# empymod/emg3d

Measured on AMD Instinct MI355X. Metric: Mcells/s per multigrid cycle, higher is better.
Workload: dtype c128

## Files before the change

### emg3d_amd/_lib.py

```python
import ctypes
import os

import numpy as np

_HERE = os.path.dirname(os.path.abspath(__file__))
LIB_PATH = os.environ.get("EMG3D_HIP_LIB") or os.path.join(_HERE, "libemg3d_hip.so")
LAB_PATH = os.path.join(_HERE, "libemg3d_hip_lab.so")

c_i64 = ctypes.c_int64
c_int = ctypes.c_int
c_vp = ctypes.c_void_p
c_double = ctypes.c_double
c_dp = ctypes.POINTER(ctypes.c_double)

ABI_VERSION = 109

SIGNATURES = {
    "emg3d_hip_version": (c_int, []),
    "emg3d_hip_device_count": (c_int, [ctypes.POINTER(c_int)]),
    "emg3d_hip_set_device": (c_int, [c_int]),
    "emg3d_hip_device_info": (c_int, [c_int, ctypes.c_char_p, ctypes.POINTER(c_i64), ctypes.POINTER(c_int)]),
    "emg3d_hip_mem_info": (c_int, [c_int, ctypes.POINTER(c_i64), ctypes.POINTER(c_i64)]),
    "emg3d_hip_release_cached": (c_i64, []),
    "emg3d_hip_cached_bytes": (c_i64, []),
    "emg3d_hip_cached_bytes_on": (c_i64, [c_int]),
    "emg3d_mg_placement": (c_int, [c_vp, c_int, ctypes.POINTER(c_int), ctypes.POINTER(c_int), ctypes.POINTER(ctypes.c_float)]),
    "emg3d_amat_x": (c_int, [c_int, c_i64, c_i64, c_i64, c_vp, c_vp, c_vp, c_vp, c_vp, c_vp, c_vp, c_vp, c_vp]),
    "emg3d_get_h_field": (c_int, [c_int, c_i64, c_i64, c_i64, c_vp, c_vp, c_vp, c_vp, c_vp, c_vp, c_double, c_double]),
    "emg3d_gauss_seidel": (c_int, [c_int, c_int, c_i64, c_i64, c_i64, c_vp, c_vp, c_vp, c_vp, c_vp, c_vp,
                                   c_vp, c_vp, c_vp, c_int, c_int]),
    "emg3d_restrict": (c_int, [c_int, c_i64, c_i64, c_i64, c_i64, c_i64, c_i64, c_vp, c_vp, c_vp, c_int]),
    "emg3d_restrict_weights": (c_int, [c_vp, c_vp, c_vp, c_i64, c_vp, c_vp, c_vp, c_i64, c_vp, c_vp, c_vp]),
    "emg3d_solve": (c_int, [c_int, c_vp, c_vp, c_i64]),
    "emg3d_blocks_to_amat": (c_int, [c_int, c_vp, c_vp, c_i64, c_vp, c_vp, c_vp, c_i64, c_i64]),
    "emg3d_prolongation": (c_int, [c_int, c_i64, c_i64, c_i64, c_vp, c_vp, c_vp, c_vp, c_vp, c_vp, c_int]),
    "emg3d_restrict_model": (c_int, [c_int, c_i64, c_i64, c_i64, c_vp, c_vp, c_int]),
    "emg3d_sweep_plan": (c_int, [c_int, c_i64, c_i64, c_i64, c_int, c_int, c_int, c_int, ctypes.c_char_p, ctypes.POINTER(c_i64)]),
    "emg3d_mg_create": (c_int, [ctypes.POINTER(c_vp), c_int, c_i64, c_i64, c_i64, c_vp, c_vp, c_vp, c_vp,
                                c_vp, c_vp, c_vp, c_vp, c_int]),
    "emg3d_mg_destroy": (None, [c_vp]),
    "emg3d_mg_create_sv": (c_int, [ctypes.POINTER(c_vp), c_int, c_i64, c_i64, c_i64, c_vp, c_vp, c_vp, c_vp,
                                   c_vp, c_vp, c_vp, c_vp, c_double, c_double, c_int]),
    "emg3d_mg_create_vs": (c_int, [ctypes.POINTER(c_vp), c_int, c_i64, c_i64, c_i64, c_vp, c_vp, c_vp, c_vp,
                                   c_vp, c_vp, c_vp, c_vp, c_vp, c_double, c_double, c_int, c_int]),
    "emg3d_mg_create_vse": (c_int, [ctypes.POINTER(c_vp), c_int, c_i64, c_i64, c_i64, c_vp, c_vp, c_vp, c_vp,
                                    c_vp, c_vp, c_vp, c_vp, c_vp, c_vp, c_double, c_double, c_double, c_int, c_int]),
    "emg3d_mg_set_smu0_eps": (c_int, [c_vp, c_double, c_double, c_double]),
    "emg3d_mg_set_sfield_vector": (c_int, [c_vp, c_vp, c_double, c_double]),
    "emg3d_mg_set_sfield_dipole": (c_int, [c_vp, c_vp, c_vp, c_int, c_int, c_vp]),
    "emg3d_source_field": (c_int, [c_int, c_i64, c_i64, c_i64, c_vp, c_vp, c_vp, c_vp, c_vp, c_vp, c_int, c_vp, c_vp]),
    "emg3d_mg_prepare": (c_int, [c_vp, c_int, c_int]),
    "emg3d_mg_set_trace": (c_int, [c_vp, c_int]),
    "emg3d_mg_get_trace": (c_int, [c_vp, c_int, c_vp, c_vp, c_vp]),
    "emg3d_mg_set_params": (c_int, [c_vp, c_int, c_int, c_int, c_int, c_int, c_vp, c_int]),
    "emg3d_mg_set_sfield": (c_int, [c_vp, c_vp]),
    "emg3d_mg_set_efield": (c_int, [c_vp, c_vp]),
    "emg3d_mg_get_efield": (c_int, [c_vp, c_vp]),
    "emg3d_mg_get_residual": (c_int, [c_vp, c_vp]),
    "emg3d_mg_get_hfield": (c_int, [c_vp, c_int, c_double, c_double, c_vp]),
    "emg3d_interp3d": (c_int, [c_int, c_i64, c_i64, c_i64, c_vp, c_vp, c_vp, c_vp, c_i64, c_vp, c_int, c_int, c_double,
                               c_double, c_vp]),
    "emg3d_get_receiver_response": (c_int, [c_int, c_i64, c_i64, c_i64, c_vp, c_vp, c_vp, c_vp, c_vp, c_int, c_i64,
                                            c_vp, c_vp, c_vp]),
    "emg3d_mg_get_receiver_response": (c_int, [c_vp, c_int, c_int, c_double, c_double, c_i64, c_vp, c_vp, c_vp]),
    "emg3d_edges2cellaverages": (c_int, [c_int, c_i64, c_i64, c_i64, c_vp, c_vp, c_vp, c_vp, c_vp]),
    "emg3d_mg_gradient": (c_int, [c_vp, c_int, c_double, c_double, c_vp]),
    "emg3d_mg_gradient3": (c_int, [c_vp, c_int, c_double, c_double, c_vp, c_vp, c_vp]),
    "emg3d_mg_grad_acc_reset": (c_int, [c_vp]),
    "emg3d_mg_grad_acc_add": (c_int, [c_vp, c_int, c_double, c_double, c_vp]),
    "emg3d_mg_grad_acc_get": (c_int, [c_vp, c_vp]),
    "emg3d_mg_grad_acc3_reset": (c_int, [c_vp]),
    "emg3d_mg_grad_acc3_add": (c_int, [c_vp, c_int, c_double, c_double, c_vp]),
    "emg3d_mg_grad_acc3_get": (c_int, [c_vp, c_vp, c_vp, c_vp]),
    "emg3d_cells2edges": (c_int, [c_int, c_i64, c_i64, c_i64, c_vp, c_vp, c_vp, c_vp, c_vp, c_vp, c_vp]),
    "emg3d_mg_jvec_source": (c_int, [c_vp, c_int, c_double, c_double, c_vp, c_vp, c_vp]),
    "emg3d_mg_jvec_source_b": (c_int, [c_vp, c_int, c_double, c_double, c_vp, c_vp, c_vp, c_vp]),
    "emg3d_mg_get_receiver_response_linear": (c_int, [c_vp, c_i64, c_vp, c_vp, c_vp]),
    "emg3d_mg_set_receiver_adjoint": (c_int, [c_vp, c_i64, c_vp, c_vp, c_vp, c_int]),
    "emg3d_mg_get_receiver_response_linear_h": (c_int, [c_vp, c_double, c_double, c_i64, c_vp, c_vp, c_vp]),
    "emg3d_mg_set_receiver_adjoint_ex": (c_int, [c_vp, c_int, c_int, c_double, c_double, c_i64, c_vp, c_vp, c_vp, c_int]),
    "emg3d_mg_set_receiver_adjoint_b": (c_int, [c_vp, c_int, c_int, c_double, c_double, c_i64, c_vp, c_vp, c_vp, c_vp, c_int]),
    "emg3d_receiver_adjoint": (c_int, [c_int, c_i64, c_i64, c_i64, c_vp, c_vp, c_vp, c_vp, c_int, c_int, c_double, c_double,
                                       c_i64, c_vp, c_vp, c_vp, c_vp]),
    "emg3d_volume_average_weights": (c_int, [c_vp, c_i64, c_vp, c_i64, c_vp, c_vp, c_vp, c_vp, c_vp]),
    "emg3d_volume_average": (c_int, [c_int, c_i64, c_i64, c_i64, c_vp, c_vp, c_vp, c_vp, c_i64, c_i64, c_i64, c_vp, c_vp,
                                     c_vp, c_vp, c_vp]),
    "emg3d_interp3d_grid": (c_int, [c_int, c_i64, c_i64, c_i64, c_vp, c_vp, c_vp, c_vp, c_i64, c_vp, c_i64, c_vp, c_i64,
                                    c_vp, c_int, c_int, c_double, c_double, c_vp]),
    "emg3d_mg_set_batch": (c_int, [c_vp, c_int]),
    "emg3d_mg_get_batch": (c_int, [c_vp]),
    "emg3d_mg_select": (c_int, [c_vp, c_int]),
    "emg3d_mg_set_mask": (c_int, [c_vp, c_vp]),
    "emg3d_mg_residual_norm": (c_int, [c_vp, c_dp]),
    "emg3d_mg_sfield_norm": (c_int, [c_vp, c_dp]),
    "emg3d_mg_smooth": (c_int, [c_vp, c_int, c_int]),
    "emg3d_mg_begin": (c_int, [c_vp, c_int]),
    "emg3d_mg_set_smu0": (c_int, [c_vp, ctypes.c_double, ctypes.c_double]),
    "emg3d_mg_cycle": (c_int, [c_vp, c_int, c_int, c_dp]),
    "emg3d_mg_cycle_next": (c_int, [c_vp, c_int, c_int, c_int, c_int, c_dp]),
    "emg3d_mg_cycles": (c_int, [c_vp, c_int, c_vp, c_int, c_vp, c_int, c_vp]),
    "emg3d_mg_efield_devptr": (c_vp, [c_vp]),
    "emg3d_mg_sfield_devptr": (c_vp, [c_vp]),
    "emg3d_mg_stream": (c_vp, [c_vp]),
    "emg3d_mg_nE": (c_i64, [c_vp]),
    "emg3d_mg_sync": (c_int, [c_vp]),
    "emg3d_mg_device_bytes": (c_i64, [c_vp]),
    "emg3d_mg_time_sweep": (c_int, [c_vp, c_int, c_int, ctypes.POINTER(ctypes.c_float)]),
    "emg3d_mg_last_sweep_kernel": (c_int, [c_vp, ctypes.c_char_p]),
    "emg3d_mg_time_residual": (c_int, [c_vp, c_int, ctypes.POINTER(ctypes.c_float)]),
    "emg3d_mg_last_residual_kernel": (c_int, [c_vp, ctypes.c_char_p]),
    "emg3d_mg_amatvec": (c_int, [c_vp, c_vp, c_vp]),
    "emg3d_mg_vec_alloc": (c_int, [c_vp, c_int]),
    "emg3d_mg_vec_set": (c_int, [c_vp, c_int, c_vp]),
    "emg3d_mg_vec_get": (c_int, [c_vp, c_int, c_vp]),
    "emg3d_mg_vec_copy": (c_int, [c_vp, c_int, c_int]),
    "emg3d_mg_vec_axpy": (c_int, [c_vp, c_int, c_double, c_double, c_int]),
    "emg3d_mg_vec_scale": (c_int, [c_vp, c_int, c_double, c_double]),
    "emg3d_mg_vec_dot": (c_int, [c_vp, c_int, c_int, c_dp]),
    "emg3d_mg_vec_amatvec": (c_int, [c_vp, c_int, c_int]),
    "emg3d_mg_bvec_alloc": (c_int, [c_vp, c_int]),
# ... 25 lines not shown
            "  python -c 'import __graft_entry__ as g; g.build()'   (needs hipcc)\n"
            "emg3d_amd has no CPU fallback.")
    lib = ctypes.CDLL(path)
    try:
        lib.emg3d_hip_version.restype = c_int
        got = int(lib.emg3d_hip_version())
    except AttributeError:
        got = None
    if got != ABI_VERSION:
        raise HipLibraryError(
            f"{path} has ABI version {got}, this package needs {ABI_VERSION} (include/emg3d_hip.h: EMG3D_HIP_ABI_VERSION): "
            "a stale build. Rebuild it with\n  python -c 'import __graft_entry__ as g; g.build(force=True)'")
    for name, (res, args) in SIGNATURES.items():
        fn = getattr(lib, name)
        fn.restype = res
        fn.argtypes = args
    _loaded[path] = lib
    return lib


def load():
    global _lib, _path
    if _lib is None:
        _lib, _path = _open(LIB_PATH), LIB_PATH
    return _lib


def use(path=None):
    global _lib, _path
    prev = _path or LIB_PATH
    want = path or LIB_PATH
    _lib, _path = _open(want), want
    return prev


def check(status, what):
    if status != 0:
        raise HipLibraryError(f"{what} failed with status {status} "
                              f"({'invalid argument' if status < 0 else 'HIP error'})")


def dtype_code(dtype):
    dtype = np.dtype(dtype)
    if dtype == np.complex128:
        return 1
    if dtype == np.float64:
        return 0
    raise TypeError(f"fields must be float64 or complex128, got {dtype}")


def ptr(a):
    return a.ctypes.data_as(c_vp)


def device_count():
    n = c_int(0)
    check(load().emg3d_hip_device_count(ctypes.byref(n)), "emg3d_hip_device_count")
    return n.value


def device_info(device=0):
    name = ctypes.create_string_buffer(256)
    mem = c_i64(0)
    cus = c_int(0)
    check(load().emg3d_hip_device_info(device, name, ctypes.byref(mem), ctypes.byref(cus)),
          "emg3d_hip_device_info")
    return {"name": name.value.decode(), "total_mem": mem.value, "cu_count": cus.value}


def mem_info(device=0):
    fr, tot = c_i64(0), c_i64(0)
    check(load().emg3d_hip_mem_info(device, ctypes.byref(fr), ctypes.byref(tot)), "emg3d_hip_mem_info")
    return {"free": fr.value, "total": tot.value, "pooled": int(load().emg3d_hip_cached_bytes()),
            "pooled_on_device": int(load().emg3d_hip_cached_bytes_on(device))}


def sweep_plan(vnC, direction, dtype=np.complex128, ordering='colour', nsys=1, cu_count=0):
    name = ctypes.create_string_buffer(64)
    info = (c_i64 * 6)()
    check(load().emg3d_sweep_plan(dtype_code(dtype), int(vnC[0]), int(vnC[1]), int(vnC[2]), int(direction),
                                  1 if ordering == 'colour' else 0, int(nsys), int(cu_count), name, info), "emg3d_sweep_plan")
    return {"kernel": name.value.decode(), "lines_per_colour": info[0], "lines_per_wave": info[1], "rounds": info[2],
            "factor_kind": info[3], "split": bool(info[4]), "big_offsets": bool(info[5])}
```

### emg3d_amd/csrc/emg3d_hip.hip

```cpp
#include "../../include/emg3d_hip.h"

#include <cstring>
#include <new>

#include <chrono>
#include "mg.hpp"
#include "receivers.hpp"
#include "source.hpp"
#include "gradient.hpp"
#include "regrid.hpp"

#define EMG3D_HIP_VERSION EMG3D_HIP_ABI_VERSION

namespace {

template <class T>
MG<T>* as(emg3d_mg_t* mg) { return static_cast<MG<T>*>(reinterpret_cast<emg3d_mg*>(mg)); }

static int current_device() { int d = 0; if (hipGetDevice(&d) != hipSuccess) { (void)hipGetLastError(); d = 0; } return d; }

template <class T> static T scalar_of(double re, double im);
template <> double scalar_of<double>(double re, double) { return re; }
template <> c128 scalar_of<c128>(double re, double im) { return mk(re, im); }

// ... 408 lines not shown
template <class T>
void receiver_components(const std::vector<double> nodes[3], const std::vector<double> centers[3], const i64 nC[3],
                         bool electric, const T* field_dev, RcvComp<T> comp[3]) {
    i64 o = 0;
    for (int c = 0; c < 3; ++c) {
        comp[c].dev = field_dev + o;
        i64 tot = 1;
        for (int a = 0; a < 3; ++a) {
            const bool cell = electric ? (a == c) : (a != c);
            comp[c].n[a] = cell ? nC[a] : nC[a] + 1;
            comp[c].pts[a] = cell ? centers[a] : nodes[a];
            tot *= comp[c].n[a];
        }
        o += tot;
    }
}

inline void grid_vectors(const double* h, i64 n, double origin, std::vector<double>& nodes, std::vector<double>& centers) {
    nodes.resize(n + 1); centers.resize(n);
    double cs = 0.0;
    nodes[0] = 0.0 + origin;
    for (i64 i = 0; i < n; ++i) { cs += h[i]; nodes[i + 1] = cs + origin; }
    for (i64 i = 0; i < n; ++i) centers[i] = (nodes[i + 1] + nodes[i]) / 2;
}

template <class T>
int receiver_host_impl(i64 nx, i64 ny, i64 nz, const double* hx, const double* hy, const double* hz, const double* origin,
                       const void* field, int is_electric, i64 n, const double* xyz, const double* fac, void* resp) {
    const i64 nC[3] = {nx, ny, nz};
    const double* hh[3] = {hx, hy, hz};
    std::vector<double> nodes[3], centers[3];
    for (int a = 0; a < 3; ++a) grid_vectors(hh[a], nC[a], origin ? origin[a] : 0.0, nodes[a], centers[a]);
    const i64 nF = is_electric ? n_edges(nC) : hfield_size(nC);
    T *df = nullptr, *scr = nullptr;
    DEV_ALLOC(df, (size_t)nF * sizeof(T));
    DEV_ALLOC(scr, (size_t)nF * sizeof(T));
    HIP_TRY(hipMemcpy(df, field, (size_t)nF * sizeof(T), hipMemcpyHostToDevice));
    RcvComp<T> comp[3];
    receiver_components<T>(nodes, centers, nC, is_electric != 0, df, comp);
    const int rc = receiver_response_device<T>(nullptr, comp, n, xyz, fac, scr, (T*)resp);
        return rc;
}

template <class T>
int interp3d_host_impl(i64 nx, i64 ny, i64 nz, const double* px, const double* py, const double* pz, const void* values,
                       i64 n, const double* xi, int method, int has_fill, double fill, double cval, void* out) {
    const i64 nn[3] = {nx, ny, nz};
    std::vector<double> pts[3];
    pts[0].assign(px, px + nx); pts[1].assign(py, py + ny); pts[2].assign(pz, pz + nz);
    const i64 tot = nx * ny * nz;
    T *dv = nullptr, *scr = nullptr, *dout = nullptr;
    DEV_ALLOC(dv, (size_t)tot * sizeof(T));
    DEV_ALLOC(scr, (size_t)tot * sizeof(T));
    DEV_ALLOC(dout, (size_t)n * sizeof(T));
    HIP_TRY(hipMemcpy(dv, values, (size_t)tot * sizeof(T), hipMemcpyHostToDevice));
    int rc = interp3d_device<T>(nullptr, dv, nn, 0, 1, nx, nx * ny, pts, n, xi, method, has_fill != 0, fill, cval, nullptr, scr, dout);
    if (rc == 0 && hipMemcpy(out, dout, (size_t)n * sizeof(T), hipMemcpyDeviceToHost) != hipSuccess) rc = (int)hipGetLastError();
        return rc;
}

}

template <class T>
static void* efield_ptr(MG<T>* m) {
    if (hipSetDevice(m->device) != hipSuccess) { (void)hipGetLastError(); return nullptr; }
    T* p = m->sel_e();
    m->check_launch();
    return m->err ? nullptr : (void*)p;
}

template <class T>
static int sweep_plan_impl(i64 nx, i64 ny, i64 nz, int dir, int order, int nsys, int cu_count, char* name, int64_t* info) {
    SweepKnobs K;
    if (cu_count > 0) K.simds = 4 * (i64)cu_count;
    else sweep_device_knobs<T>(K, current_device());
    K.order = order; K.nsys = nsys;
    const SweepPlan p = plan_sweep(K, SweepShape{{nx, ny, nz}, (int)sizeof(T)}, dir - 1);
    memcpy(name, p.name, sizeof p.name);
    info[0] = p.nmax; info[1] = p.lpw; info[2] = p.rounds; info[3] = p.fac_kind; info[4] = p.split ? 1 : 0; info[5] = p.big ? 1 : 0;
    return 0;
}

template <class T>
static int jvec_stage(MG<T>* m, const double* const hv[3], const double* dv[3]) {
    Level<T>& L = *m->lv0;
    double* stage = reinterpret_cast<double*>(L.r);
    const i64 n = L.nCells;
    int used = 0;
    for (int c = 0; c < 3; ++c) {
        dv[c] = nullptr;
        if (!hv[c]) continue;
        for (int q = 0; q < c; ++q) if (hv[q] == hv[c]) dv[c] = dv[q];
        if (dv[c]) continue;
        double* d = stage + (i64)used++ * n;
        HIP_TRY(hipMemcpyAsync(d, hv[c], (size_t)n * sizeof(double), hipMemcpyHostToDevice, m->stream));
        dv[c] = d;
    }
    return 0;
}

template <class T>
static int jvec_source_impl(MG<T>* m, int efield_vec, double smu0_re, double smu0_im, const double* vx, const double* vy,
                            const double* vz) {
    if (sizeof(T) == 8 && smu0_im != 0.0) return -2;
    HIP_TRY(hipSetDevice(m->device));
    Level<T>& L = *m->lv0;
    const T* fwd = m->vec(efield_vec);
    if (!fwd || efield_vec < 0) return -2;
    const double* hv[3] = {vx, vy, vz};
    const double* dv[3];
    { const int st = jvec_stage<T>(m, hv, dv); if (st) return st; }
    T* s = m->sel_s();
    if (m->broken) return (int)hipErrorOutOfMemory;
    hipLaunchKernelGGL(k_jvec_source<T>, dim3((unsigned)((L.nE + 255) / 256)), dim3(256), 0, m->stream, L.nC[0], L.nC[1], L.nC[2],
                       L.fl, fwd, smu0_re, smu0_im, dv[0], dv[1], dv[2], (const double*)L.h[0], (const double*)L.h[1],
                       (const double*)L.h[2], s, L.nE);
    m->source_changed();
    m->lv0->s_dense = true;
    m->check_launch();
    return finish(m);
}

template <class T>
static int jvec_source_b_impl(MG<T>* m, int fwd_bvec, double smu0_re, double smu0_im, const double* vx, const double* vy,
                              const double* vz, const int32_t* use) {
    if (sizeof(T) == 8 && smu0_im != 0.0) return -2;
    HIP_TRY(hipSetDevice(m->device));
    Level<T>& L = *m->lv0;
    if (fwd_bvec < 0 || fwd_bvec >= (int)m->bvecs.size()) return -2;
    const T* fwd = m->bvecs[(size_t)fwd_bvec];
    unsigned long long bits = 0;
    for (int b = 0; b < m->nsys; ++b) if (use[b]) bits |= 1ull << b;
    if (!bits) return 0;
    const double* hv[3] = {vx, vy, vz};
    const double* dv[3];
    { const int st = jvec_stage<T>(m, hv, dv); if (st) return st; }
    if (m->broken) return (int)hipErrorOutOfMemory;
    hipLaunchKernelGGL(k_jvec_source_b<T>, dim3((unsigned)((L.nE + 255) / 256)), dim3(256), 0, m->stream, L.nC[0], L.nC[1], L.nC[2],
                       L.fl, fwd, m->nsys, bits, smu0_re, smu0_im, dv[0], dv[1], dv[2], (const double*)L.h[0], (const double*)L.h[1],
                       (const double*)L.h[2], L.s, L.nE);
    m->source_changed();
    m->lv0->s_dense = true;
    m->check_launch();
    return finish(m);
}

static int gradient_impl(emg3d_mg_t* mg, int efield_vec, double smu0_re, double smu0_im, double* gx, double* gy, double* gz) {
    const bool split = gy != nullptr;
    DISPATCH(mg, {
        HIP_TRY(hipSetDevice(m->device));
        Level<T>& L = *m->lv0;
        const T* fwd = m->vec(efield_vec);
        if (!fwd || efield_vec == -2) return -2;
        double* dg = reinterpret_cast<double*>(L.r);
        const i64 n = L.nCells;
        const unsigned blocks = (unsigned)((n + 255) / 256);
        const T* bwd = m->sel_e();
        if (m->broken) return (int)hipErrorOutOfMemory;
        if (split)
            hipLaunchKernelGGL((k_gradient<T, true>), dim3(blocks), dim3(256), 0, m->stream, L.nC[0], L.nC[1], L.nC[2], L.fl, fwd, bwd,
                               smu0_re, smu0_im, (const double*)L.h[0], (const double*)L.h[1], (const double*)L.h[2], dg, dg + n, dg + 2 * n);
        else
            hipLaunchKernelGGL((k_gradient<T, false>), dim3(blocks), dim3(256), 0, m->stream, L.nC[0], L.nC[1], L.nC[2], L.fl, fwd, bwd,
                               smu0_re, smu0_im, (const double*)L.h[0], (const double*)L.h[1], (const double*)L.h[2], dg, (double*)nullptr,
                               (double*)nullptr);
        m->check_launch();
// ... 164 lines not shown
}

int emg3d_hip_mem_info(int device, int64_t* free_bytes, int64_t* total_bytes) {
    int prev = 0;
    HIP_TRY(hipGetDevice(&prev));
    HIP_TRY(hipSetDevice(device));
    size_t fr = 0, tot = 0;
    const hipError_t e = hipMemGetInfo(&fr, &tot);
    (void)hipSetDevice(prev);
    if (e != hipSuccess) { (void)hipGetLastError(); return (int)e; }
    if (free_bytes) *free_bytes = (int64_t)fr;
    if (total_bytes) *total_bytes = (int64_t)tot;
    return 0;
}

int emg3d_amat_x(int dtype, int64_t nx, int64_t ny, int64_t nz, void* r, const void* e, const void* eta_x,
                 const void* eta_y, const void* eta_z, const double* zeta, const double* hx,
                 const double* hy, const double* hz) {
    return dtype ? amat_x_impl<c128>(nx, ny, nz, r, e, eta_x, eta_y, eta_z, zeta, hx, hy, hz)
                 : amat_x_impl<double>(nx, ny, nz, r, e, eta_x, eta_y, eta_z, zeta, hx, hy, hz);
}

int emg3d_get_h_field(int dtype, int64_t nx, int64_t ny, int64_t nz, void* hfield, const void* efield,
                      const double* zeta, const double* hx, const double* hy, const double* hz,
                      double smu0_re, double smu0_im) {
    if (nx < 1 || ny < 1 || nz < 1 || !hfield || !efield || !hx || !hy || !hz) return -2;
    if (smu0_re == 0.0 && smu0_im == 0.0) return -2;
    if (!dtype && smu0_im != 0.0) return -2;
    return dtype ? hfield_impl<c128>(nx, ny, nz, hfield, efield, zeta, hx, hy, hz, smu0_re, smu0_im)
                 : hfield_impl<double>(nx, ny, nz, hfield, efield, zeta, hx, hy, hz, smu0_re, smu0_im);
}

int emg3d_gauss_seidel(int dtype, int dir, int64_t nx, int64_t ny, int64_t nz, void* e, const void* s,
                       const void* eta_x, const void* eta_y, const void* eta_z, const double* zeta,
                       const double* hx, const double* hy, const double* hz, int nu, int order) {
    return dtype ? gs_impl<c128>(dir, nx, ny, nz, e, s, eta_x, eta_y, eta_z, zeta, hx, hy, hz, nu, order)
                 : gs_impl<double>(dir, nx, ny, nz, e, s, eta_x, eta_y, eta_z, zeta, hx, hy, hz, nu, order);
}

int emg3d_restrict(int dtype, int64_t nx, int64_t ny, int64_t nz, int64_t cnx, int64_t cny, int64_t cnz,
                   void* cr, const void* r, const double* const* w, int sc_dir) {
    return dtype ? restrict_impl<c128>(nx, ny, nz, cnx, cny, cnz, cr, r, w, sc_dir)
                 : restrict_impl<double>(nx, ny, nz, cnx, cny, cnz, cr, r, w, sc_dir);
}

int emg3d_restrict_weights(const double* vectorN, const double* vectorCC, const double* h, int64_t nh,
                           const double* cvectorN, const double* cvectorCC, const double* ch, int64_t n,
                           double* wl, double* w0, double* wr) {
    if (n < 2 || nh < 2) return -2;
    restrict_weights_host(vectorN, vectorCC, h, nh, cvectorN, cvectorCC, ch, n, wl, w0, wr);
    return 0;
}

int emg3d_solve(int dtype, void* amat, void* bvec, int64_t n) {
    if (n < 1) return -2;
    return dtype ? solve_impl<c128>(amat, bvec, n) : solve_impl<double>(amat, bvec, n);
}

int emg3d_blocks_to_amat(int dtype, void* amat, void* bvec, int64_t n, const void* middle, const double* left,
                         const void* rhs, int64_t im, int64_t nC) {
    return dtype ? b2a_impl<c128>(amat, bvec, n, middle, left, rhs, im, nC)
                 : b2a_impl<double>(amat, bvec, n, middle, left, rhs, im, nC);
}

int emg3d_prolongation(int dtype, int64_t nx, int64_t ny, int64_t nz, const double* hx, const double* hy,
                       const double* hz, const double* origin, void* e, const void* ce, int sc_dir) {
    return dtype ? prolong_impl<c128>(nx, ny, nz, hx, hy, hz, origin, e, ce, sc_dir)
                 : prolong_impl<double>(nx, ny, nz, hx, hy, hz, origin, e, ce, sc_dir);
}

int emg3d_restrict_model(int is_complex, int64_t nx, int64_t ny, int64_t nz, void* cparam, const void* param,
                         int sc_dir) {
    return is_complex ? restrict_model_impl<c128>(nx, ny, nz, cparam, param, sc_dir)
                      : restrict_model_impl<double>(nx, ny, nz, cparam, param, sc_dir);
}

int emg3d_sweep_plan(int dtype, int64_t nx, int64_t ny, int64_t nz, int dir, int order, int nsys, int cu_count, char* name,
                     int64_t* info) {
    if (nx < 2 || ny < 2 || nz < 2 || dir < 1 || dir > 3 || order < 0 || order > 1 || nsys < 1 || nsys > 64 || !name || !info) return -2;
    return dtype ? sweep_plan_impl<c128>(nx, ny, nz, dir, order, nsys, cu_count, name, info)
                 : sweep_plan_impl<double>(nx, ny, nz, dir, order, nsys, cu_count, name, info);
}

int emg3d_mg_create(emg3d_mg_t** out, int dtype, int64_t nx, int64_t ny, int64_t nz, const double* hx,
                    const double* hy, const double* hz, const double* origin, const void* eta_x,
                    const void* eta_y, const void* eta_z, const double* zeta, int device) {
    if (!out) return -1;
    return dtype ? create_impl<c128>(out, 1, nx, ny, nz, hx, hy, hz, origin, eta_x, eta_y, eta_z, zeta, device)
                 : create_impl<double>(out, 0, nx, ny, nz, hx, hy, hz, origin, eta_x, eta_y, eta_z, zeta, device);
}

int emg3d_mg_create_sv(emg3d_mg_t** out, int dtype, int64_t nx, int64_t ny, int64_t nz, const double* hx,
                       const double* hy, const double* hz, const double* origin, const double* sv_x,
                       const double* sv_y, const double* sv_z, const double* zeta, double smu0_re,
                       double smu0_im, int device) {
    if (!out || !sv_x) return -1;
    return dtype ? create_impl<c128>(out, 1, nx, ny, nz, hx, hy, hz, origin, sv_x, sv_y, sv_z, zeta, device, true, smu0_re, smu0_im)
                 : create_impl<double>(out, 0, nx, ny, nz, hx, hy, hz, origin, sv_x, sv_y, sv_z, zeta, device, true, smu0_re, smu0_im);
}

int emg3d_mg_create_vs(emg3d_mg_t** out, int dtype, int64_t nx, int64_t ny, int64_t nz, const double* hx,
                       const double* hy, const double* hz, const double* origin, const double* sigma_x,
                       const double* sigma_y, const double* sigma_z, const double* vol, const double* zeta,
                       double smu0_re, double smu0_im, int resistivity, int device) {
    if (!out || !sigma_x || !vol) return -1;
    if (dtype ? smu0_re != 0.0 : smu0_im != 0.0) return -2;
    return dtype ? create_impl<c128>(out, 1, nx, ny, nz, hx, hy, hz, origin, sigma_x, sigma_y, sigma_z, zeta, device, true, smu0_re, smu0_im, vol, resistivity != 0)
                 : create_impl<double>(out, 0, nx, ny, nz, hx, hy, hz, origin, sigma_x, sigma_y, sigma_z, zeta, device, true, smu0_re, smu0_im, vol, resistivity != 0);
}

int emg3d_mg_create_vse(emg3d_mg_t** out, int dtype, int64_t nx, int64_t ny, int64_t nz, const double* hx,
                        const double* hy, const double* hz, const double* origin, const double* sigma_x,
                        const double* sigma_y, const double* sigma_z, const double* vol, const double* zeta,
                        const double* epsilon_r, double smu0_re, double smu0_im, double seps0, int resistivity, int device) {
    if (!out || !sigma_x || !vol || !epsilon_r) return -1;
    if (dtype ? smu0_re != 0.0 : smu0_im != 0.0) return -2;
    return dtype ? create_impl<c128>(out, 1, nx, ny, nz, hx, hy, hz, origin, sigma_x, sigma_y, sigma_z, zeta, device, true, smu0_re, smu0_im, vol, resistivity != 0, epsilon_r, seps0)
                 : create_impl<double>(out, 0, nx, ny, nz, hx, hy, hz, origin, sigma_x, sigma_y, sigma_z, zeta, device, true, smu0_re, smu0_im, vol, resistivity != 0, epsilon_r, seps0);
}

void emg3d_mg_destroy(emg3d_mg_t* mg) {
    if (!mg) return;
    const bool broken = reinterpret_cast<emg3d_mg*>(mg)->dtype ? as<c128>(mg)->broken : as<double>(mg)->broken;
    delete reinterpret_cast<emg3d_mg*>(mg);
    if (broken) (void)hipGetLastError();
}

int emg3d_mg_set_params(emg3d_mg_t* mg, int cycle, int nu_init, int nu_pre, int nu_coarse, int nu_post,
                        const int* clevel, int order) {
    if (cycle != 'V' && cycle != 'W' && cycle != 'F') return -2;
    if (order != 0 && order != 1) return -2;
    DISPATCH(mg, {
        bool same = m->cycle == cycle && m->nu_init == nu_init && m->nu_pre == nu_pre && m->nu_coarse == nu_coarse &&
                    m->nu_post == nu_post && m->order == order;
        if (clevel) for (int q = 0; q < 4; ++q) same = same && m->clevel[q] == clevel[q];
        if (!same) m->drop_graphs();
        m->cycle = cycle; m->cycmax = (cycle == 'V') ? 1 : 2;
        m->entry_cm = 0;
        m->nu_init = nu_init; m->nu_pre = nu_pre; m->nu_coarse = nu_coarse; m->nu_post = nu_post;
        if (clevel) {
            bool changed = false;
            for (int q = 0; q < 4; ++q) { if (m->clevel[q] != clevel[q]) changed = true; m->clevel[q] = clevel[q]; }
            if (changed) m->hier.clear();
        }
        if (m->order != order) {
            HIP_TRY(hipSetDevice(m->device));
            m->e_to_ref(*m->lv0);
            m->check_launch();
            m->order = order;
            m->forget_factors();
        }
        return 0;
    });
}

int emg3d_mg_set_smu0(emg3d_mg_t* mg, double smu0_re, double smu0_im) {
    DISPATCH(mg, {
        HIP_TRY(hipSetDevice(m->device));
        if (sizeof(T) == 8 && smu0_im != 0.0) return -2;
        if (sizeof(T) == 16 && m->volw && smu0_re != 0.0) return -2;
        if (m->epsr) return -7;
        const int st = m->set_smu0(scalar_of<T>(smu0_re, smu0_im));
        if (st) return st;
        return finish(m);
    });
}
// ... 669 lines not shown
```

### emg3d_amd/csrc/mg.hpp

```cpp
#pragma once
#include <algorithm>
#include <cmath>
#include <cstdlib>
#include <cstring>
#include <map>
#include <memory>
#include <mutex>
#include <chrono>
#include <vector>

#include "common.hpp"
#include "smooth.hpp"
#include "stencil.hpp"
#include "gradient.hpp"
#include "smooth_qpl.hpp"
#include "smooth_qc.hpp"
#include "smooth_thm.hpp"
#include "smooth_tha.hpp"
#include "sweep_launch.hpp"
#include "sweep_plan.hpp"

template <class T>
struct Level {
    i64 nC[3];
    i64 nE, nCells;
    FieldLayout fl;
    CellLayout cl;
    std::vector<double> h_host[3], nodes[3], centers[3];
    double* h[3] = {nullptr, nullptr, nullptr};
    double* ih[3] = {nullptr, nullptr, nullptr};
    T* eta[3] = {nullptr, nullptr, nullptr};
    double* zeta = nullptr;
    unsigned char* sflag[3] = {nullptr, nullptr, nullptr};
    bool sflag_valid[3] = {false, false, false};
    bool s_dense = false;
    bool zeta_sep = false;
    T *s = nullptr, *e = nullptr, *r = nullptr;
    T *eT = nullptr, *sT = nullptr;
    T* etaT[3] = {nullptr, nullptr, nullptr};
    double* zetaT = nullptr;
    bool sT_valid = false;
    FieldLayout flT;
    CellLayout clT;
    T *eW[2] = {nullptr, nullptr}, *sW[2] = {nullptr, nullptr};
    double* zetaW[2] = {nullptr, nullptr};
    bool sW_valid[2] = {false, false};
    int e_home = 0;
    T* fac[3] = {nullptr, nullptr, nullptr};
    void* qd[3][4] = {{nullptr, nullptr, nullptr, nullptr}, {nullptr, nullptr, nullptr, nullptr}, {nullptr, nullptr, nullptr, nullptr}};
    unsigned qdn[3][4] = {{0, 0, 0, 0}, {0, 0, 0, 0}, {0, 0, 0, 0}};
    i64 fac_lines[3] = {0, 0, 0};
    i64 fac_mid[3] = {0, 0, 0};
    int fac_kind[3] = {0, 0, 0};
    SweepPlan plan[3];
    int plan_key[3] = {-1, -1, -1};
};

struct Transfer {
    int sc = -1;
    int co[3] = {0, 0, 0};
    double* w[3][3] = {{nullptr, nullptr, nullptr}, {nullptr, nullptr, nullptr}, {nullptr, nullptr, nullptr}};
    int* pidx[3] = {nullptr, nullptr, nullptr};
    double* pwt[3] = {nullptr, nullptr, nullptr};
};

template <class T>
struct Hierarchy {
    std::vector<std::shared_ptr<Level<T>>> lv;
    std::vector<Transfer> tr;
};

class DevicePool {
    std::mutex mu;
    struct Parked { void* p; int tag; };
    std::multimap<std::pair<int, size_t>, Parked> free_blocks;
    size_t held = 0, cap;
public:
    DevicePool() {
        const char* g = getenv("EMG3D_POOL_GB");
        cap = (size_t)((g ? atof(g) : 96.0) * (double)((size_t)1 << 30));
    }
    void* take(int device, size_t nb, int tag = 0, bool* hit = nullptr) {
        std::lock_guard<std::mutex> lk(mu);
        if (hit) *hit = false;
        auto rng = free_blocks.equal_range({device, nb});
        if (rng.first == rng.second) return nullptr;
        auto pick = rng.second;
        for (auto it = rng.first; it != rng.second; ++it) if (it->second.tag == tag) { pick = it; break; }
        if (pick == rng.second && tag != 0)
            for (auto it = rng.first; it != rng.second; ++it) if (it->second.tag == 0) { pick = it; break; }
        if (pick == rng.second) pick = rng.first;
        if (hit) *hit = tag != 0 && pick->second.tag == tag;
        void* p = pick->second.p;
        free_blocks.erase(pick);
        held -= nb;
        return p;
    }
    bool give(int device, void* p, size_t nb, int tag = 0) {
        std::lock_guard<std::mutex> lk(mu);
        if (held + nb > cap) return false;
        free_blocks.insert({{device, nb}, Parked{p, tag}});
        held += nb;
        return true;
    }
    size_t release_all() {
        std::lock_guard<std::mutex> lk(mu);
        const size_t n = held;
        int cur = 0;
        (void)hipGetDevice(&cur);
        for (auto& kv : free_blocks) {
            if (kv.first.first < 0) { (void)hipHostFree(kv.second.p); continue; }
            (void)hipSetDevice(kv.first.first); (void)hipFree(kv.second.p);
        }
        for (auto& kv : free_streams) { (void)hipSetDevice(kv.first); (void)hipStreamDestroy(kv.second); }
        free_streams.clear();
        (void)hipSetDevice(cur);
        free_blocks.clear();
        held = 0;
        return n;
    }
    size_t bytes_held() { std::lock_guard<std::mutex> lk(mu); return held; }
    size_t bytes_held_on(int device) {
        std::lock_guard<std::mutex> lk(mu);
        size_t n = 0;
        for (auto& kv : free_blocks) if (kv.first.first == device) n += kv.first.second;
        return n;
    }
    std::multimap<int, hipStream_t> free_streams;
    hipStream_t take_stream(int device) {
        {
            std::lock_guard<std::mutex> lk(mu);
            auto it = free_streams.find(device);
            if (it != free_streams.end()) { hipStream_t s = it->second; free_streams.erase(it); return s; }
// ... 808 lines not shown
            if (L.eta[c] == L.eta[0]) { L.etaT[c] = L.etaT[0]; continue; }
            L.etaT[c] = dalloc<T>(L.nCells);
            transpose_xy(L.etaT[c], (const T*)L.eta[c], L.nC[0], L.nC[1], L.nC[2], true, 0);
        }
        L.zetaT = dalloc<double>(L.nCells);
        transpose_xy(L.zetaT, (const double*)L.zeta, L.nC[0], L.nC[1], L.nC[2], true, 0);
        L.sT_valid = false;
    }
    void ensure_work(Level<T>& L, int w) {
        if (L.eW[w]) return;
        if (&L == lv0.get() && place_applies(L) && !placed[w]) {
            want_tag = 1 + w;
            L.eW[w] = dalloc<T>(nsys * L.nE);
            want_tag = 0;
            if (L.eW[w] && got_tag) { placed[w] = true; block_tag[L.eW[w]] = 1 + w; place_rec[w] = PlaceRec(); place_rec[w].reused = 1; }
        } else
        L.eW[w] = dalloc<T>(nsys * L.nE);
        L.sW[w] = dalloc<T>(nsys * L.nE);
        L.zetaW[w] = dalloc<double>(L.nCells);
        if (w == 1) split_x(L.zetaW[w], (const double*)L.zeta, L.nC[0], L.nC[1] * L.nC[2], true);
        else transpose_xy(L.zetaW[w], (const double*)L.zeta, L.nC[0], L.nC[1], L.nC[2], true, 1);
        L.sW_valid[w] = false;
    }
    bool split_on(Level<T>& L) { return plan(L, 0).split; }
    int use_home = (int)LAB_ENV("EMG3D_HOME", 1);
    bool home_on(Level<T>& L) { return use_home && &L == lv0.get() && split_on(L); }
    bool home_lvl(Level<T>& L) { return use_home && &L != lv0.get() && split_on(L); }
    void e_to_ref(Level<T>& L) {
        if (L.e_home != 1) return;
        convert_field(L, L.e, L.eW[1], 1, false, true);
        L.e_home = 0;
    }
    void e_to_w1(Level<T>& L) {
        if (L.e_home == 1) return;
        ensure_work(L, 1);
        convert_field(L, L.eW[1], L.e, 1, true, true);
        L.e_home = 1;
    }

    int lex_loop = (int)LAB_ENV("EMG3D_LEX_LOOP", 1);
    void line_args(Level<T>& L, int dir, LineArgs<T>& a, bool sweep) {
        if (dir == 0) { a.L = 0; a.P = 1; a.Q = 2; }
        else if (dir == 1) { a.L = 1; a.P = 0; a.Q = 2; }
        else { a.L = 2; a.P = 0; a.Q = 1; }
        const SweepPlan& P = plan(L, dir);
        const bool sp = sweep && P.split;
        const bool t = (sp && dir == 0) ? true : P.xt;
        const int w = (dir == 0) ? 0 : 1;
        for (int q = 0; q < 3; ++q) {
            a.nC[q] = L.nC[q]; a.eta[q] = t ? L.etaT[q] : L.eta[q]; a.h[q] = L.h[q]; a.ih[q] = L.ih[q];
        }
        a.fl = t ? L.flT : L.fl; a.cl = t ? L.clT : L.cl;
        a.split = sp ? 1 : 0;
        if (sp) { a.e = L.eW[w]; a.s = L.sW[w]; a.zeta = L.zetaW[w]; }
        else { a.e = t ? L.eT : L.e; a.s = t ? L.sT : L.s; a.zeta = t ? L.zetaT : L.zeta; }
        const i64 nP = L.nC[a.P], nQ = L.nC[a.Q];
        a.nA[0] = (nP - 0) / 2; a.nA[1] = (nP - 1) / 2;
        const i64 nB[2] = {(nQ - 0) / 2, (nQ - 1) / 2};
        a.nB2[0] = nB[0]; a.nB2[1] = nB[1];
        i64 o = 0;
        for (int c = 0; c < 4; ++c) { a.base[c] = o; o += a.nA[c & 1] * nB[c >> 1]; }
        a.nLinesTot = o;
        a.fac = L.fac[dir];
        a.mid = L.fac[dir] ? L.fac_mid[dir] : L.nC[a.L] - 1;
        a.qm = (L.fac[dir] && L.fac_kind[dir] == 3) ? 2 : 0;
        a.fcomp = (L.fac[dir] && L.fac_kind[dir] == 4) ? 1 : 0;
        a.zsep = (sweep && L.zeta_sep && use_zsep) ? 1 : 0;
        a.sflag = (sweep && sflag_on(L, dir) && L.sflag[dir] && L.sflag_valid[dir]) ? L.sflag[dir] : nullptr;
        a.xcd = xcd_map;
        a.tile = q_tile;
        {
            const int ax[3] = {a.L, a.P, a.Q};
            a.rs.ihL = a.ih[a.L]; a.rs.ihP = a.ih[a.P]; a.rs.ihQ = a.ih[a.Q];
            a.rs.hL = a.h[a.L]; a.rs.hP = a.h[a.P]; a.rs.hQ = a.h[a.Q];
            a.rs.nL = (unsigned)a.nC[a.L]; a.rs.slot0 = 0;
            a.rs.nP = (unsigned)a.nC[a.P]; a.rs.nQ = (unsigned)a.nC[a.Q];
            a.rs.csL = (unsigned)a.cl.st[a.L]; a.rs.csP = (unsigned)a.cl.st[a.P]; a.rs.csQ = (unsigned)a.cl.st[a.Q];
            for (int c = 0; c < 3; ++c) {
                a.rs.off[c] = (unsigned)a.fl.off[ax[c]];
                for (int d = 0; d < 3; ++d) a.rs.st[c][d] = (unsigned)a.fl.st[ax[c]][ax[d]];
            }
        }
        a.qd = nullptr; a.qdn = 0;
        a.qpl = P.NW; a.qM = P.M; a.seg = P.seg; a.qlpw = 0;
        a.tha = P.helpers;
        a.mode = 0; a.cP = a.cQ = 0; a.cntA = a.cntB = 0; a.t = a.jQ0 = a.cnt = 0;
        a.bt = sweep ? batch(L) : Batch();
    }

    void ensure_factor(Level<T>& L, int dir) {
        const SweepPlan& P = plan(L, dir);
        if (P.xt) ensure_transposed_model(L);
        if (L.fac[dir]) return;
        L.fac_lines[dir] = (L.nC[dir == 0 ? 1 : 0] - 1) * (L.nC[dir == 2 ? 1 : 2] - 1);
        L.fac[dir] = dalloc<T>(L.fac_lines[dir] * P.fac_entries);
        L.fac_mid[dir] = P.mid;
        L.fac_kind[dir] = P.fac_kind;
        if (P.fac_kind == 3) thm_attrs();
        compute_factor(L, dir);
    }
    void compute_factor(Level<T>& L, int dir) {
        LineArgs<T> a;
        line_args(L, dir, a, false);
        a.fac = L.fac[dir];
        a.fcomp = L.fac_kind[dir] == 4;
        if (L.fac_kind[dir] == 3) {
            a.mid = L.fac_mid[dir];
            const i64 nQ_ = L.nC[a.Q];
            const i64 nmax_ = a.nA[0] * ((nQ_ - 0) / 2);
            a.mode = 3;
            if (nmax_ > 0)
                MG_LAUNCH(k_line_factor_m<T>, dim3((unsigned)((nmax_ + EMG_LINE_BLOCK - 1) / EMG_LINE_BLOCK), 4),
                                   dim3(EMG_LINE_BLOCK), 0, stream, a);
            check_launch();
            return;
        }
        a.mid = L.fac_mid[dir];
        const i64 nQ = L.nC[a.Q];
        const i64 nB[2] = {(nQ - 0) / 2, (nQ - 1) / 2};
        a.mode = 3; a.cP = a.cQ = 0; a.cntA = a.cntB = 0;
        const i64 nmax = a.nA[0] * nB[0];
#ifdef EMG3D_LAB
        if (LAB_ENV("EMG3D_FACTOR_PER_COLOUR", 0)) {
            for (int c = 0; c < 4; ++c) {
                a.mode = 0; a.cP = c & 1; a.cQ = c >> 1; a.cntA = a.nA[a.cP]; a.cntB = nB[a.cQ];
                const i64 n = a.cntA * a.cntB;
                if (n > 0)
                    MG_LAUNCH(k_line_factor<T>, dim3((unsigned)((n + EMG_LINE_BLOCK - 1) / EMG_LINE_BLOCK)),
                                       dim3(EMG_LINE_BLOCK), 0, stream, a);
            }
            check_launch();
            return;
        }
#endif
        if (nmax > 0)
            MG_LAUNCH(k_line_factor<T>, dim3((unsigned)((nmax + EMG_LINE_BLOCK - 1) / EMG_LINE_BLOCK), 4),
                               dim3(EMG_LINE_BLOCK), 0, stream, a);
        check_launch();
    }

    unsigned xcd_grid(i64 nb) const { return (unsigned)(xcd_map ? ((nb + 7) / 8) * 8 : nb); }
    unsigned rp_grid(i64 nt) const { return xcd_grid((nt + EMG_RP_BLOCK - 1) / EMG_RP_BLOCK); }
    void ensure_qdesc(Level<T>& L, int dir) {
        const SweepPlan& P = plan(L, dir);
        if (!P.qdesc || L.qd[dir][0] || L.qdn[dir][0] == ~0u) return;
        L.qdn[dir][0] = ~0u;
        if (!L.fac[dir]) return;
        LineArgs<T> a;
        line_args(L, dir, a, true);
        const i64 lpg = 16 / a.seg;
        a.bt = Batch();
        for (int c = 0; c < 4; ++c) {
            a.mode = 0; a.cP = c & 1; a.cQ = c >> 1;
            a.cntA = a.nA[a.cP]; a.cntB = a.nB2[a.cQ];
            a.rs.slot0 = (unsigned)a.base[c];
            const i64 n = a.cntA * a.cntB;
            if (n <= 0) continue;
            const unsigned grid = xcd_grid((n + lpg - 1) / lpg);
            const i64 nthreads = (i64)grid * 64;
            void* tab = try_alloc<char>(nthreads * a.qM * (3 * 16 + 8 * 16));
            if (!tab) return;
            a.qd = tab; a.qdn = (unsigned)nthreads;
            if (!broken) qpl_launch<T>(1, a.qM, false, 1, false, dim3(grid), stream, a);
            L.qd[dir][c] = tab; L.qdn[dir][c] = (unsigned)nthreads;
        }
        check_launch();
// ... 108 lines not shown
    bool placement_pending(int lr_dir) {
        Level<T>& L = *lv0;
        if (!place_applies(L)) return false;
        const int lr = current_lr_dir(lr_dir, L.nC);
        return (lr_has(lr, 0) && !placed[0]) || ((lr_has(lr, 1) || lr_has(lr, 2)) && !placed[1]);
    }
    bool alloc_quiet = false;
    template <class U>
    U* try_alloc(i64 n) {
        const int keep = err;
        const i64 keep_bytes = bytes;
        alloc_quiet = true;
        U* p = dalloc<U>(n);
        alloc_quiet = false;
        if (!p) { err = keep; bytes = keep_bytes; }
        return p;
    }
    float time_sweeps(Level<T>& L, int dir, int reps) {
        hipEvent_t t0 = nullptr, t1 = nullptr;
        float ms = -1.f;
        if (hipEventCreate(&t0) == hipSuccess && hipEventCreate(&t1) == hipSuccess && hipEventRecord(t0, stream) == hipSuccess) {
            for (int i = 0; i < reps; ++i) smooth_line(L, dir, 1, false, false);
            if (hipEventRecord(t1, stream) == hipSuccess && hipEventSynchronize(t1) == hipSuccess &&
                hipEventElapsedTime(&ms, t0, t1) == hipSuccess) ms /= (float)reps;
            else ms = -1.f;
        }
        if (ms < 0.f) (void)hipGetLastError();
        if (t0) hipEventDestroy(t0);
        if (t1) hipEventDestroy(t1);
        return ms;
    }
    void place_level0(int lr_dir) {
        Level<T>& L = *lv0;
        if (dry || !placement_pending(lr_dir)) return;
        const int lr = current_lr_dir(lr_dir, L.nC);
        bool moved = false;
        for (int w = 0; w < 2; ++w) {
            const int dir = (w == 0) ? (lr_has(lr, 0) ? 0 : -1) : lr_has(lr, 1) ? 1 : lr_has(lr, 2) ? 2 : -1;
            if (placed[w] || dir < 0 || !L.eW[w] || !L.sW[w] || !L.fac[dir]) continue;
            placed[w] = true;
            if (w == 1) e_to_ref(L);
            if (!L.sW_valid[w]) { convert_field(L, L.sW[w], L.s, w, true); L.sW_valid[w] = true; }
            ensure_sflags(L, dir);
            const i64 n = (i64)nsys * L.nE;
            PlaceRec& R = place_rec[w];
            R = PlaceRec();
            T* cands[PLACE_MAX];
            cands[0] = L.eW[w];
            int best = 0;
            float worst = 0.f;
            const int nt = std::min<int>(place_tries, PLACE_MAX);
            for (int k = 0; k < nt; ++k) {
                T* c = (k == 0) ? cands[0] : try_alloc<T>(n);
                if (!c) break;
                cands[k] = c;
                hipMemsetAsync(c, 0, (size_t)n * sizeof(T), stream);
                L.eW[w] = c;
                if (k == 0) (void)time_sweeps(L, dir, 1);
                const float ms = time_sweeps(L, dir, place_reps);
                R.ms[k] = ms;
                R.tries = k + 1;
                if (ms < 0.f) break;
                if (ms < R.ms[best]) best = k;
                worst = std::max(worst, ms);
                if ((double)R.ms[best] * place_gap < (double)worst) break;
            }
            if (R.ms[best] < 0.f) best = 0;
            R.kept = best;
            L.eW[w] = cands[best];
            block_tag[cands[best]] = 1 + w;
            for (int k = 0; k < R.tries; ++k) if (k != best) release(cands[k]);
            moved |= best != 0;
            if (getenv("EMG3D_LOG_SETUP")) {
                fprintf(stderr, "[place] working copy %d (%s-lines, %.0f MB): kept candidate %d of %d;", w, dir == 0 ? "x" : dir == 1 ? "y" : "z",
                        (double)n * sizeof(T) / 1048576.0, best, R.tries);
                for (int k = 0; k < R.tries; ++k) fprintf(stderr, " %.3f", R.ms[k]);
                fprintf(stderr, " ms per sweep\n");
            }
        }
        if (moved) drop_graphs();
        check_launch();
    }

    void smooth_line(Level<T>& L, int dir, int nu, bool conv_in = true, bool conv_out = true) {
        if (nu <= 0) return;
        ensure_factor(L, dir);
        ensure_qdesc(L, dir);
        if (dry) { prepare_work(L, dir); return; }
        if (conv_in) to_work(L, dir);
        ensure_sflags(L, dir);
        LineArgs<T> a;
        line_args(L, dir, a, true);
        const SweepPlan& P = plan(L, dir);
        const i64 nP = L.nC[a.P], nQ = L.nC[a.Q];
        const i64 nB[2] = {(nQ - 0) / 2, (nQ - 1) / 2};
        int iback = 0;
        int last_c = -1;
        for (int it = 0; it < nu; ++it) {
            iback = 1 - iback;
            if (order == 1) {
                for (int ch = 0; ch < 4; ++ch) {
                    const int c = iback ? colour_perm_b[ch] : colour_perm[ch];
                    if (skip_idempotent && c == last_c) continue;
                    last_c = c;
                    a.mode = 0; a.cP = c & 1; a.cQ = c >> 1;
                    a.cntA = a.nA[a.cP]; a.cntB = nB[a.cQ];
                    a.rs.slot0 = (unsigned)a.base[c];
                    a.qd = L.qd[dir][c]; a.qdn = (L.qd[dir][c] ? L.qdn[dir][c] : 0u);
                    const i64 n = a.cntA * a.cntB;
                    if (n <= 0) continue;
                    launch_sweep(P, a, n);
                }
            } else {
                const i64 tmin = 3, tmax = (nP - 1) + 2 * (nQ - 1);
                if (lex_loop && a.qpl && a.qM == 1 && a.seg <= 16) {
                    LineArgs<T> b = a;
                    b.mode = 2; b.t = tmin; b.jQ0 = tmax; b.cnt = iback; b.xcd = 0;
                    const i64 maxn = std::min<i64>(nQ - 1, (nP - 1) / 2 + 1), quads = maxn * a.seg;
                    const int lnw = quads <= 16 ? 1 : quads <= 32 ? 2 : quads <= 64 ? 4 : 8;
                    if (!broken) qpl_launch<T>(lnw, 1, true, 0, false, bgrid(1), stream, b);
                    sweep_kernel_name(sweep_name, sizeof sweep_name, SweepFamily::qpl, (int)sizeof(T), lnw, 1);
                    continue;
                }
                for (i64 th = tmin; th <= tmax; ++th) {
                    const i64 tt = iback ? tmax - (th - tmin) : th;
                    i64 lo = tt - (nP - 1);
                    i64 jQ0 = lo <= 0 ? 1 : (lo + 1) / 2;
                    if (jQ0 < 1) jQ0 = 1;
                    i64 jQ1 = (tt - 1) / 2;
                    if (jQ1 > nQ - 1) jQ1 = nQ - 1;
                    const i64 n = jQ1 - jQ0 + 1;
                    if (n <= 0) continue;
                    a.mode = 1; a.t = tt; a.jQ0 = jQ0; a.cnt = n;
                    launch_sweep(P, a, n);
                }
            }
        }
        if (conv_out) from_work(L, dir);
        check_launch();
    }

    void smooth_point(Level<T>& L, int nu) {
        if (dry) return;
        if (&L == lv0.get()) e_to_ref(L);
        const bool hl = home_lvl(L) && L.e_home == 1;
        if (hl) { convert_field(L, L.e, L.eW[1], 1, false); convert_field(L, L.s, L.sW[1], 1, false); }
        PointArgs<T> a;
        for (int q = 0; q < 3; ++q) { a.nC[q] = L.nC[q]; a.eta[q] = L.eta[q]; a.h[q] = L.h[q]; a.ih[q] = L.ih[q]; }
        a.fl = L.fl; a.e = L.e; a.s = L.s; a.zeta = L.zeta; a.bt = batch(L);
        a.col = 0; a.t = 0; a.cnt[0] = a.cnt[1] = a.cnt[2] = 0;
        int iback = 0;
        int last_c = -1;
        for (int it = 0; it < nu; ++it) {
            iback = 1 - iback;
            if (order == 1) {
                for (int ch = 0; ch < 8; ++ch) {
                    const int c = iback ? point_perm_b[ch] : point_perm[ch];
                    if (skip_idempotent && c == last_c) continue;
                    last_c = c;
                    a.mode = 0; a.col = c;
                    for (int q = 0; q < 3; ++q) a.cnt[q] = (L.nC[q] - ((c >> q) & 1)) / 2;
                    const i64 n = a.cnt[0] * a.cnt[1] * a.cnt[2];
                    if (n <= 0) continue;
                    MG_LAUNCH(k_point_sweep<T>, bgrid_y((unsigned)((n + EMG_LINE_BLOCK - 1) / EMG_LINE_BLOCK)),
                                       dim3(EMG_LINE_BLOCK), 0, stream, a);
                }
            } else {
                const i64 tmin = 7, tmax = (L.nC[0] - 1) + 2 * (L.nC[1] - 1) + 4 * (L.nC[2] - 1);
                const i64 n = (L.nC[1] - 1) * (L.nC[2] - 1);
                for (i64 th = tmin; th <= tmax; ++th) {
                    a.mode = 1; a.t = iback ? tmax - (th - tmin) : th;
                    MG_LAUNCH(k_point_sweep<T>, bgrid_y((unsigned)((n + EMG_LINE_BLOCK - 1) / EMG_LINE_BLOCK)),
                                       dim3(EMG_LINE_BLOCK), 0, stream, a);
                }
            }
        }
        if (hl) convert_field(L, L.eW[1], L.e, 1, true);
        check_launch();
    }

    void smoothing(Level<T>& L, int nu, int lr_dir) {
        const int lr = current_lr_dir(lr_dir, L.nC);
        if (lr == 0) smooth_point(L, nu);
        int dirs[3], nd = 0;
        if (lr == 1 || lr == 5 || lr == 6 || lr == 7) dirs[nd++] = 0;
        if (lr == 2 || lr == 4 || lr == 6 || lr == 7) dirs[nd++] = 1;
        if (lr == 3 || lr == 4 || lr == 5 || lr == 7) dirs[nd++] = 2;
        for (int k = 0; k < nd; ++k) {
            const bool in = (k == 0) || work_id(L, dirs[k - 1]) != work_id(L, dirs[k]);
            const bool out = (k == nd - 1) || work_id(L, dirs[k + 1]) != work_id(L, dirs[k]);
            smooth_line(L, dirs[k], nu, in, out);
        }
    }

    void residual(Level<T>& L, int mode, int slot) {
        ResidualArgs<T> a;
// ... 120 lines not shown
    void refresh_level0_source() {
        Level<T>& L = *lv0;
        if (L.sT && !L.sT_valid) { convert_field(L, L.sT, L.s, -1, true); L.sT_valid = true; }
        for (int w = 0; w < 2; ++w)
            if (L.sW[w] && !L.sW_valid[w]) { convert_field(L, L.sW[w], L.s, w, true); L.sW_valid[w] = true; }
        for (int d = 0; d < 3; ++d)
            if (L.sflag[d]) ensure_sflags(L, d);
    }

    void prepare(int g, int lr_dir) {
        if (!use_graph) { dry = true; cycle0_eager(g, lr_dir, 0); dry = false; place_level0(lr_dir); return; }
        cycle0(g, lr_dir, -1);
    }

    void cycle0(int g, int lr_dir, int slot) {
        if (!use_graph || trace) {
            if (slot >= 0) {
                if (placement_pending(lr_dir)) prepare(g, lr_dir);
                cycle0_eager(g, lr_dir, slot);
            }
            return;
        }
        const int key = (g * 8 + lr_dir) * 4 + entry_cm;
        auto it = graphs.find(key);
        if (it != graphs.end() && slot < 0) return;
        const int home_in = (home_on(*lv0) && current_lr_dir(lr_dir, lv0->nC) != 0) ? 1 : 0;
        if (it == graphs.end()) {
            const bool tlog = getenv("EMG3D_LOG_SETUP") != nullptr;
            auto now = [] { return std::chrono::steady_clock::now(); };
            auto ms = [](auto a, auto b) { return std::chrono::duration<double, std::milli>(b - a).count(); };
            auto t0 = now();
            const size_t nalloc0 = allocs.size();
            dry = true;
            cycle0_eager(g, lr_dir, 0);
            dry = false;
            place_level0(lr_dir);
            const int home_keep = (slot >= 0) ? home_in : lv0->e_home;
            if (slot >= 0) { if (home_in) e_to_w1(*lv0); else e_to_ref(*lv0); }
            else if (home_in) ensure_work(*lv0, 1);
            lv0->e_home = home_in;
            refresh_level0_source();
            if (tlog) hipStreamSynchronize(stream);
            auto t1 = now();
            hipGraph_t graph = nullptr;
            hipGraphExec_t exec = nullptr;
            hipError_t st = hipStreamBeginCapture(stream, hipStreamCaptureModeThreadLocal);
            if (st == hipSuccess) {
                cycle0_eager(g, lr_dir, 0);
                st = hipStreamEndCapture(stream, &graph);
            }
            const int home_out = lv0->e_home;
            lv0->e_home = home_keep;
            auto t2 = now();
            if (st == hipSuccess) st = hipGraphInstantiate(&exec, graph, nullptr, nullptr, 0);
            if (graph) hipGraphDestroy(graph);
            if (tlog) fprintf(stderr, "[setup] key %d: hierarchy+factors %.2f ms (%zu allocations), capture %.2f ms, instantiate %.2f ms\n",
                              key, ms(t0, t1), allocs.size() - nalloc0, ms(t1, t2), ms(t2, now()));
            if (st != hipSuccess || err != 0) {
                (void)hipGetLastError();
                fprintf(stderr, "[emg3d_hip] hipGraph capture failed (%s); using eager launches\n", hipGetErrorString(st));
                use_graph = false;
                err = 0;
                if (slot >= 0) cycle0_eager(g, lr_dir, slot);
                return;
            }
            (void)hipGraphUpload(exec, stream);
            graphs[key] = exec;
            graph_home[key] = std::make_pair(home_in, home_out);
            it = graphs.find(key);
            if (slot < 0) return;
        }
        const std::pair<int, int> hm = graph_home[key];
        if (hm.first) e_to_w1(*lv0); else e_to_ref(*lv0);
        refresh_level0_source();
        hipError_t st = hipGraphLaunch(it->second, stream);
        if (st != hipSuccess && err == 0) err = (int)st;
        lv0->e_home = hm.second;
        if (slot != 0) hipMemcpyAsync(norms + (i64)slot * nsys, norms, (size_t)nsys * sizeof(double), hipMemcpyDeviceToDevice, stream);
    }

    void forget_factors() {
        auto clear = [](Level<T>& L) {
            for (int d = 0; d < 3; ++d) {
                L.fac[d] = nullptr; L.fac_kind[d] = 0; L.plan_key[d] = -1;
                for (int c = 0; c < 4; ++c) { L.qd[d][c] = nullptr; L.qdn[d][c] = 0; }
            }
        };
        if (lv0) clear(*lv0);
        for (auto& kv : hier) for (auto& l : kv.second.lv) if (l) clear(*l);
    }

    void drop_graphs() {
        for (auto& kv : graphs) hipGraphExecDestroy(kv.second);
        graphs.clear();
        graph_home.clear();
        graph_seen.clear();
    }
};
```

### emg3d_amd/csrc/smooth.hpp

```cpp
#pragma once
#include "common.hpp"

#define EMG_LINE_BLOCK 64

template <class T>
struct LineArgs {
    int L, P, Q;
    i64 nC[3];
    FieldLayout fl;
    CellLayout cl;
    T* e;
    const T* s;
    const T* eta[3];
    const double* zeta;
    const double* h[3];
    const double* ih[3];
    int split;
    i64 mid;
    int xcd;
    int tile;
    struct Resolved {
        const double *ihL, *ihP, *ihQ;
        const double *hL, *hP, *hQ;
        unsigned nL, csL, csP, csQ;
        unsigned nP, nQ;
        unsigned slot0;
        unsigned off[3], st[3][3];
    } rs;
    Batch bt;
    int qm;
    int qpl;
    int qM, seg;
    const unsigned char* sflag;
    int zsep;
    int qlpw;
    int tha;
    int fcomp;
    T* fac;
    const void* qd;
    unsigned qdn;
    i64 nLinesTot;
    i64 base[4];
    i64 nA[2];
    i64 nB2[2];
    int mode;
    int cP, cQ;
    i64 cntA, cntB;
    i64 t, jQ0, cnt;
};

template <class T>
__device__ __forceinline__ bool line_of_thread(const LineArgs<T>& a, i64& jP, i64& jQ) {
    const i64 idx = (i64)blockIdx.x * blockDim.x + threadIdx.x;
    if (a.mode == 0) {
        if (idx >= a.cntA * a.cntB) return false;
        const i64 b = idx / a.cntA, q = idx - b * a.cntA;
        jP = 1 + a.cP + 2 * q;
        jQ = 1 + a.cQ + 2 * b;
    } else {
        if (idx >= a.cnt) return false;
        jQ = a.jQ0 + idx;
        jP = a.t - 2 * jQ;
    }
    return true;
}

template <class T>
__device__ __forceinline__ i64 line_slot(const LineArgs<T>& a, i64 jP, i64 jQ) {
    const int cP = (int)((jP - 1) & 1), cQ = (int)((jQ - 1) & 1);
    return a.base[cP + 2 * cQ] + ((jP - 1) >> 1) + a.nA[cP] * ((jQ - 1) >> 1);
}

struct LineCoef {
    double QP_Lm[2], PQ_Lm[2];
    double QL_Pm[2], LQ_Pm[2], QL_Pp[2], LQ_Pp[2];
    double PL_Qm[2], LP_Qm[2], PL_Qp[2], LP_Qp[2];
};

__device__ __forceinline__ void line_coef(LineCoef& c, const double z[2][2][2], const double kL[2],
                                          const double kP[2], const double kQ[2]) {
#pragma unroll
    for (int S = 0; S < 2; ++S) {
        c.QP_Lm[S] = kP[S] * (z[0][S][1] + z[0][S][0]);
        c.PQ_Lm[S] = kQ[S] * (z[0][1][S] + z[0][0][S]);
        c.QL_Pm[S] = kL[S] * (z[S][0][1] + z[S][0][0]);
        c.LQ_Pm[S] = kQ[S] * (z[1][0][S] + z[0][0][S]);
        c.QL_Pp[S] = kL[S] * (z[S][1][1] + z[S][1][0]);
        c.LQ_Pp[S] = kQ[S] * (z[1][1][S] + z[0][1][S]);
        c.PL_Qm[S] = kL[S] * (z[S][1][0] + z[S][0][0]);
        c.LP_Qm[S] = kP[S] * (z[1][S][0] + z[0][S][0]);
        c.PL_Qp[S] = kL[S] * (z[S][1][1] + z[S][0][1]);
        c.LP_Qp[S] = kP[S] * (z[1][S][1] + z[0][S][1]);
    }
}

__device__ __forceinline__ void line_left(const LineCoef& c, double ihLm, double a[5], double d[5]) {
    a[0] = 0.0; d[0] = 0.0;
    a[1] = c.QP_Lm[0] * ihLm;
    a[2] = -c.QP_Lm[1] * ihLm;
    a[3] = c.PQ_Lm[0] * ihLm;
    a[4] = -c.PQ_Lm[1] * ihLm;
    d[1] = -c.QL_Pm[0] * ihLm;
    d[2] = -c.QL_Pp[0] * ihLm;
    d[3] = -c.PL_Qm[0] * ihLm;
    d[4] = -c.PL_Qp[0] * ihLm;
}

__host__ __device__ __forceinline__ constexpr int wpk(int r, int c) {
    return r >= c ? r * (r + 1) / 2 + c : c * (c + 1) / 2 + r;
}

template <class T>
__device__ __forceinline__ void apply_sinv(const T f[15], T y[5]) {
    T o[5];
#pragma unroll
    for (int r = 0; r < 5; ++r) {
        T t = f[wpk(r, 0)] * y[0];
#pragma unroll
        for (int c = 1; c < 5; ++c) t += f[wpk(r, c)] * y[c];
        o[r] = t;
    }
#pragma unroll
    for (int r = 0; r < 5; ++r) y[r] = o[r];
// ... 1101 lines not shown
```

### emg3d_amd/csrc/smooth_qpl.hpp

```cpp
#pragma once
#include "smooth.hpp"


template <int K>
__device__ __forceinline__ double quad_bcast(double v) {
    constexpr int ctrl = K | (K << 2) | (K << 4) | (K << 6);
    int lo = __double2loint(v), hi = __double2hiint(v);
    lo = __builtin_amdgcn_update_dpp(0, lo, ctrl, 0xf, 0xf, false);
    hi = __builtin_amdgcn_update_dpp(0, hi, ctrl, 0xf, 0xf, false);
    return __hiloint2double(hi, lo);
}
template <int K>
__device__ __forceinline__ c128 quad_bcast(c128 v) { return mk(quad_bcast<K>(v.re), quad_bcast<K>(v.im)); }
__device__ __forceinline__ double quad_sum(double v) {
    int lo = __double2loint(v), hi = __double2hiint(v);
    double o = __hiloint2double(__builtin_amdgcn_update_dpp(0, hi, 0xb1, 0xf, 0xf, false),
                                __builtin_amdgcn_update_dpp(0, lo, 0xb1, 0xf, 0xf, false));
    v += o;
    lo = __double2loint(v); hi = __double2hiint(v);
    o = __hiloint2double(__builtin_amdgcn_update_dpp(0, hi, 0x4e, 0xf, 0xf, false),
                         __builtin_amdgcn_update_dpp(0, lo, 0x4e, 0xf, 0xf, false));
    return v + o;
}
__device__ __forceinline__ c128 quad_sum(c128 v) { return mk(quad_sum(v.re), quad_sum(v.im)); }

template <bool UP>
__device__ __forceinline__ double row_shift4(double v) {
    constexpr int ctrl = UP ? 0x114 : 0x104;
    int lo = __double2loint(v), hi = __double2hiint(v);
    lo = __builtin_amdgcn_update_dpp(0, lo, ctrl, 0xf, 0xf, false);
    hi = __builtin_amdgcn_update_dpp(0, hi, ctrl, 0xf, 0xf, false);
    return __hiloint2double(hi, lo);
}
template <bool UP> __device__ __forceinline__ c128 row_shift4(c128 v) { return mk(row_shift4<UP>(v.re), row_shift4<UP>(v.im)); }
template <bool UP> __device__ __forceinline__ double lane_shift4(double v) { return UP ? __shfl_up(v, 4) : __shfl_down(v, 4); }
template <bool UP> __device__ __forceinline__ c128 lane_shift4(c128 v) { return mk(lane_shift4<UP>(v.re), lane_shift4<UP>(v.im)); }

template <class T>
__device__ __forceinline__ void qpl_args_burst(const LineArgs<T>& a) {
    asm volatile("" :: "s"(a.e), "s"(a.s), "s"(a.fac), "s"(a.zeta), "s"(a.rs.ihL), "s"(a.rs.ihP), "s"(a.rs.ihQ), "s"(a.bt.st),
                 "s"(a.bt.mask), "s"(a.bt.n), "s"(a.xcd), "s"(a.mode), "s"(a.cntA), "s"(a.cntB), "s"(a.cP), "s"(a.cQ), "s"(a.seg),
                 "s"(a.rs.nL), "s"(a.rs.csL), "s"(a.rs.csP), "s"(a.rs.csQ), "s"(a.rs.slot0), "s"(a.rs.off[0]), "s"(a.rs.off[1]),
                 "s"(a.rs.off[2]));
    asm volatile("" :: "s"(a.rs.st[0][0]), "s"(a.rs.st[0][1]), "s"(a.rs.st[0][2]), "s"(a.rs.st[1][0]), "s"(a.rs.st[1][1]),
                 "s"(a.rs.st[1][2]), "s"(a.rs.st[2][0]), "s"(a.rs.st[2][1]), "s"(a.rs.st[2][2]), "s"(a.t), "s"(a.jQ0), "s"(a.cnt),
                 "s"(a.rs.nP), "s"(a.rs.nQ), "s"(a.qd), "s"(a.qdn));
}

template <class T, int NW, int M, bool HL = false, int DM = 0, bool CH = false>
__global__ __launch_bounds__(64 * NW) void k_line_sweep_qpl(LineArgs<T> a) {
    static_assert(DM == 0 || (!HL && NW == 1), "descriptors: one wave per workgroup, colour order");
    static_assert(!CH || (NW == 1 && M == 1 && !HL), "chain form: lines inside one wave, one block per quad");
    constexpr int NQ = 16 * NW;
#ifdef EMG3D_LAB
    long long qts[7] = {0, 0, 0, 0, 0, 0, 0};
#define QPL_TS(i) do { if (a.tile & 512) { asm volatile("" ::: "memory"); qts[i] = (long long)__builtin_readcyclecounter(); asm volatile("" ::: "memory"); } } while (0)
#else
#define QPL_TS(i) do {} while (0)
#endif
    QPL_TS(0);
    qpl_args_burst(a);
    QPL_TS(1);
    const int tid = threadIdx.x;
    const int quad = tid >> 2, r = tid & 3;
    const int seg = a.seg;
    const int ch = quad & (seg - 1);
    const int lseg = __builtin_ctz((unsigned)seg);
    const int lpg = NQ >> lseg;
    typedef unsigned int u32;
    EMG_SWEEP_WG(a)
    __shared__ T xb[2][NQ][4][5];
    auto one = [&](const u32 gline, const u32 nlines, const u32 t_, const u32 jQ0_) {
    const bool live = gline < nlines;
    const int nL = (int)a.rs.nL;
    auto ld_d = [](const double* base, u32 idx) -> double { return *reinterpret_cast<const double*>(reinterpret_cast<const char*>(base) + idx * 8u); };
    auto ld_t = [](const T* base, u32 idx) -> T { return *reinterpret_cast<const T*>(reinterpret_cast<const char*>(base) + idx * (u32)sizeof(T)); };
    const T* __restrict__ e = (a.e + boff_);
    const T* __restrict__ s = (a.s + boff_);
    T Wr[M][5], W0[M][5];
    T b[M][5];
    double av[M][4], dv[M][4];
    bool lastb[M], inl[M];
    u32 dS[M], dS0[M];
    const u32 tix = (u32)wg * (64u * NW) + (u32)tid;
    constexpr int QD_U4 = 3, QD_D2 = 8;
    if constexpr (DM == 2) {
        const uint4* const q4 = reinterpret_cast<const uint4*>(a.qd);
        const emg_d2* const c2 = reinterpret_cast<const emg_d2*>(q4 + (size_t)(QD_U4 * M) * a.qdn);
        uint4 u[M][QD_U4];
        emg_d2 cf[M][QD_D2];
#pragma unroll
        for (int j = 0; j < M; ++j) {
#pragma unroll
            for (int k = 0; k < QD_U4; ++k) u[j][k] = q4[(u32)(QD_U4 * j + k) * a.qdn + tix];
#pragma unroll
            for (int k = 0; k < QD_D2; ++k) cf[j][k] = c2[(u32)(QD_D2 * j + k) * a.qdn + tix];
        }
        QPL_TS(2);
        T E[M][6], S[M], E0[M], S0[M];
#pragma unroll
        for (int j = 0; j < M; ++j) {
            const u32 oE[6] = {u[j][0].x, u[j][0].y, u[j][0].z, u[j][0].w, u[j][1].x, u[j][1].y};
            dS[j] = u[j][1].z; dS0[j] = u[j][2].x;
            inl[j] = (u[j][2].z & 1u) != 0; lastb[j] = (u[j][2].z & 2u) != 0;
            const T* w = a.fac + u[j][2].y;
#pragma unroll
            for (int c = 0; c < 5; ++c) W0[j][c] = w[(u32)(wpk(0, c) * (M * seg))];
#pragma unroll
            for (int c = 0; c < 5; ++c) {
                const int e1 = wpk(1, c), e2 = wpk(2, c), e3 = wpk(3, c), e4 = wpk(4, c);
                const int en = (r == 0) ? e1 : (r == 1) ? e2 : (r == 2) ? e3 : e4;
                Wr[j][c] = w[(u32)(en * (M * seg))];
            }
#pragma unroll
            for (int t = 0; t < 6; ++t) E[j][t] = ld_t(e, oE[t]);
            S[j] = ld_t(s, dS[j]);
            E0[j] = ld_t(e, u[j][1].w);
            S0[j] = ld_t(s, dS0[j]);
        }
#pragma unroll
        for (int j = 0; j < M; ++j) {
            const double cE[6] = {cf[j][0].x, cf[j][0].y, cf[j][1].x, cf[j][1].y, cf[j][2].x, cf[j][2].y};
            av[j][0] = cf[j][3].y; av[j][1] = cf[j][4].x; av[j][2] = cf[j][4].y; av[j][3] = cf[j][5].x;
            dv[j][0] = cf[j][5].y; dv[j][1] = cf[j][6].x; dv[j][2] = cf[j][6].y; dv[j][3] = cf[j][7].x;
            T y = S[j];
#pragma unroll
            for (int t = 0; t < 6; ++t) cmac(y, E[j][t], cE[t]);
            const T bo = lastb[j] ? Zero<T>::v() : y;
            T part = E0[j] * cf[j][3].x;
            part = quad_sum(part);
            b[j][0] = S0[j] + part;
            b[j][1] = quad_bcast<0>(bo); b[j][2] = quad_bcast<1>(bo); b[j][3] = quad_bcast<2>(bo); b[j][4] = quad_bcast<3>(bo);
            if (!inl[j]) {
#pragma unroll
                for (int c = 0; c < 5; ++c) { Wr[j][c] = Zero<T>::v(); W0[j][c] = Zero<T>::v(); }
            }
        }
    } else {
    const u32 gidx = live ? gline : 0u;
    u32 jP, jQ;
    if (a.mode == 0) {
        const u32 cA = (u32)a.cntA;
        const u32 bq = gidx / cA, qq = gidx - bq * cA;
        jP = 1u + (u32)a.cP + 2u * qq;
        jQ = 1u + (u32)a.cQ + 2u * bq;
    } else {
        jQ = jQ0_ + gidx;
        jP = t_ - 2u * jQ;
    }
    const u32 slot = (a.mode == 0) ? a.rs.slot0 + gidx : (u32)line_slot(a, (i64)jP, (i64)jQ);
    const u32 csL = a.rs.csL, csP = a.rs.csP, csQ = a.rs.csQ;
    const double ihP[2] = {ld_d(a.rs.ihP, jP - 1u), ld_d(a.rs.ihP, jP)};
    const double ihQ[2] = {ld_d(a.rs.ihQ, jQ - 1u), ld_d(a.rs.ihQ, jQ)};
    const bool tp = r < 2;
    const int side = r & 1;
    const double sg = side ? -1.0 : 1.0;
    const u32 jA = tp ? jP : jQ, jB = tp ? jQ : jP;
    const u32 acell = jA - 1u + (u32)side;
    const u32 anode = side ? jA + 1u : jA - 1u;
    const u32 oLc = a.rs.off[0], oAc = tp ? a.rs.off[1] : a.rs.off[2], oBc = tp ? a.rs.off[2] : a.rs.off[1];
    const u32 sLL = a.rs.st[0][0];
    const u32 sLA = tp ? a.rs.st[0][1] : a.rs.st[0][2], sLB = tp ? a.rs.st[0][2] : a.rs.st[0][1];
    const u32 sAL = tp ? a.rs.st[1][0] : a.rs.st[2][0];
    const u32 sAA = tp ? a.rs.st[1][1] : a.rs.st[2][2], sAB = tp ? a.rs.st[1][2] : a.rs.st[2][1];
    const u32 sBL = tp ? a.rs.st[2][0] : a.rs.st[1][0];
    const u32 sBA = tp ? a.rs.st[2][1] : a.rs.st[1][2], sBB = tp ? a.rs.st[2][2] : a.rs.st[1][1];
    u32 ob[7], os[7];
    ob[0] = oAc + sAL + acell * sAA + jB * sAB;
    ob[1] = oLc + sLL + anode * sLA + jB * sLB;
    ob[2] = ob[1] - sLL;
    ob[3] = oBc + sBL + anode * sBA + jB * sBB;
    ob[4] = ob[3] - sBB;
    ob[5] = ob[0] + sAB;
    ob[6] = ob[0] - sAB;
    os[0] = sAL; os[1] = sLL; os[2] = sLL; os[3] = sBL; os[4] = sBL; os[5] = sAL; os[6] = sAL;
    const u32 sLP = a.rs.st[0][1], sLQ = a.rs.st[0][2];
    const u32 o0 = oLc + jP * sLP + jQ * sLQ;
    const u32 db0 = (r < 2) ? sLP : sLQ;
    const u32 ob0 = (r & 1) ? o0 - db0 : o0 + db0;
// ... 29 lines not shown
        n0[j] = ld_d(a.zeta, cface + cnext + pa); n1[j] = ld_d(a.zeta, cface + cnext + pa + pb);
        ihl0[j] = ld_d(a.rs.ihL, (u32)ic); ihl1[j] = ld_d(a.rs.ihL, (u32)(lastb[j] ? ic : ic + 1));
        const u32 ie = (u32)(lastb[j] ? (ic > 0 ? ic - 1 : 0) : ic);
#pragma unroll
        for (int t = 0; t < 6; ++t) dE[j][t] = ob[1 + t] + ie * os[1 + t];
        dS[j] = ob[0] + ie * os[0];
        dE0[j] = ob0 + (u32)ic * sLL;
        dS0[j] = o0 + (u32)ic * sLL;
        if constexpr (DM == 0) {
#pragma unroll
            for (int t = 0; t < 6; ++t) E[j][t] = ld_t(e, dE[j][t]);
            S[j] = ld_t(s, dS[j]);
            E0[j] = ld_t(e, dE0[j]);
            S0[j] = ld_t(s, dS0[j]);
        }
    }
    QPL_TS(2);
    const double kP[2] = {0.5 * ihP[0], 0.5 * ihP[1]};
    const double kQ[2] = {0.5 * ihQ[0], 0.5 * ihQ[1]};
    double Kc[6];
    {
        const double ihA = tp ? (side ? ihP[1] : ihP[0]) : (side ? ihQ[1] : ihQ[0]);
        const double kB0 = tp ? kQ[0] : kP[0], kB1 = tp ? kQ[1] : kP[1];
        const double ihB0 = tp ? ihQ[0] : ihP[0], ihB1 = tp ? ihQ[1] : ihP[1];
        Kc[0] = sg * ihA; Kc[1] = -sg * ihA;
        Kc[2] = sg * kB1 * ihA; Kc[3] = -sg * kB0 * ihA;
        Kc[4] = kB1 * ihB1; Kc[5] = kB0 * ihB0;
    }
    const double K0 = (r == 0) ? kP[1] * ihP[1] : (r == 1) ? kP[0] * ihP[0] : (r == 2) ? kQ[1] * ihQ[1] : kQ[0] * ihQ[0];
#pragma unroll
    for (int j = 0; j < M; ++j) {
        const int i = ch * M + j;
        const double pP0 = f00[j] + f01[j], pP1 = f10[j] + f11[j], pQ0 = f00[j] + f10[j], pQ1 = f01[j] + f11[j];
        const double act = (i > 0 && i < nL) ? 1.0 : 0.0;
        const double t1 = act * ihl0[j], t2 = -0.5 * t1 * ihl0[j];
        av[j][0] = kP[0] * pP0 * t1; av[j][1] = -kP[1] * pP1 * t1; av[j][2] = kQ[0] * pQ0 * t1; av[j][3] = -kQ[1] * pQ1 * t1;
        dv[j][0] = t2 * pP0; dv[j][1] = t2 * pP1; dv[j][2] = t2 * pQ0; dv[j][3] = t2 * pQ1;
        double cE[6];
        {
            const double z0 = (type == 1) ? (side ? f10[j] : f00[j]) : (side ? f01[j] : f00[j]);
            const double z1 = (type == 1) ? (side ? f11[j] : f01[j]) : (side ? f11[j] : f10[j]);
            const double kL0 = 0.5 * ihl0[j], kL1 = 0.5 * ihl1[j];
            const double rs0 = z0 + z1, rs1 = n0[j] + n1[j];
            const double cs0 = z0 + n0[j], cs1 = z1 + n1[j];
            cE[0] = (Kc[0] * kL1) * rs1; cE[1] = (Kc[1] * kL0) * rs0;
            cE[2] = Kc[2] * cs1; cE[3] = Kc[3] * cs0; cE[4] = Kc[4] * cs1; cE[5] = Kc[5] * cs0;
        }
        const double c0 = K0 * ((r == 0) ? pP1 : (r == 1) ? pP0 : (r == 2) ? pQ1 : pQ0);
        if constexpr (DM == 1) {
            uint4* const q4 = reinterpret_cast<uint4*>(const_cast<void*>(a.qd));
            emg_d2* const c2 = reinterpret_cast<emg_d2*>(q4 + (size_t)(QD_U4 * M) * a.qdn);
            const u32 flags = (inl[j] ? 1u : 0u) | (lastb[j] ? 2u : 0u) | (live ? 4u : 0u);
            q4[(u32)(QD_U4 * j + 0) * a.qdn + tix] = make_uint4(dE[j][0], dE[j][1], dE[j][2], dE[j][3]);
            q4[(u32)(QD_U4 * j + 1) * a.qdn + tix] = make_uint4(dE[j][4], dE[j][5], dS[j], dE0[j]);
            q4[(u32)(QD_U4 * j + 2) * a.qdn + tix] = make_uint4(dS0[j], dF[j], flags, 0u);
            auto d2 = [](double x, double y) { emg_d2 v; v.x = x; v.y = y; return v; };
            c2[(u32)(QD_D2 * j + 0) * a.qdn + tix] = d2(cE[0], cE[1]);
            c2[(u32)(QD_D2 * j + 1) * a.qdn + tix] = d2(cE[2], cE[3]);
            c2[(u32)(QD_D2 * j + 2) * a.qdn + tix] = d2(cE[4], cE[5]);
            c2[(u32)(QD_D2 * j + 3) * a.qdn + tix] = d2(c0, av[j][0]);
            c2[(u32)(QD_D2 * j + 4) * a.qdn + tix] = d2(av[j][1], av[j][2]);
            c2[(u32)(QD_D2 * j + 5) * a.qdn + tix] = d2(av[j][3], dv[j][0]);
            c2[(u32)(QD_D2 * j + 6) * a.qdn + tix] = d2(dv[j][1], dv[j][2]);
            c2[(u32)(QD_D2 * j + 7) * a.qdn + tix] = d2(dv[j][3], 0.0);
        } else {
            T y = S[j];
#pragma unroll
            for (int t = 0; t < 6; ++t) cmac(y, E[j][t], cE[t]);
            const T bo = lastb[j] ? Zero<T>::v() : y;
            T part = E0[j] * c0;
            part = quad_sum(part);
            b[j][0] = S0[j] + part;
            b[j][1] = quad_bcast<0>(bo); b[j][2] = quad_bcast<1>(bo); b[j][3] = quad_bcast<2>(bo); b[j][4] = quad_bcast<3>(bo);
            if (!inl[j]) {
#pragma unroll
                for (int c = 0; c < 5; ++c) { Wr[j][c] = Zero<T>::v(); W0[j][c] = Zero<T>::v(); }
            }
        }
    }
    if constexpr (DM == 1) return;
    }

    QPL_TS(3);
    auto sync = [&]() { if (NW > 1 && (HL || seg > 16)) __syncthreads(); else __builtin_amdgcn_wave_barrier(); };
    T mc, mG[4];
    auto publish = [&](int p) {
        xb[p][quad][r][0] = mc;
#pragma unroll
        for (int k = 0; k < 4; ++k) xb[p][quad][r][1 + k] = mG[k];
    };
    auto compose_with = [&](int p, int src) {
        const T g0 = mG[0], g1 = mG[1], g2 = mG[2], g3 = mG[3];
        if (NW >= 4 || M > 1) {
            T n0, n1, n2, n3;
#pragma unroll
            for (int k = 0; k < 4; ++k) {
                T row[5];
#pragma unroll
                for (int j = 0; j < 5; ++j) row[j] = xb[p][src][k][j];
                const T g = (k == 0) ? g0 : (k == 1) ? g1 : (k == 2) ? g2 : g3;
                cmac(mc, g, row[0]);
                if (k == 0) { n0 = g * row[1]; n1 = g * row[2]; n2 = g * row[3]; n3 = g * row[4]; }
                else { cmac(n0, g, row[1]); cmac(n1, g, row[2]); cmac(n2, g, row[3]); cmac(n3, g, row[4]); }
                __builtin_amdgcn_sched_barrier(0);
            }
            mG[0] = n0; mG[1] = n1; mG[2] = n2; mG[3] = n3;
        } else {
            T oc[4], oG[4][4];
#pragma unroll
            for (int k = 0; k < 4; ++k) {
                oc[k] = xb[p][src][k][0];
#pragma unroll
                for (int cc = 0; cc < 4; ++cc) oG[k][cc] = xb[p][src][k][1 + cc];
            }
            cmac(mc, g0, oc[0]); cmac(mc, g1, oc[1]); cmac(mc, g2, oc[2]); cmac(mc, g3, oc[3]);
#pragma unroll
            for (int cc = 0; cc < 4; ++cc) {
                T t = g0 * oG[0][cc];
                cmac(t, g1, oG[1][cc]); cmac(t, g2, oG[2][cc]); cmac(t, g3, oG[3][cc]);
                mG[cc] = t;
            }
        }
    };
    auto compose_c_only = [&](int p, int src) {
        cmac(mc, mG[0], xb[p][src][0][0]); cmac(mc, mG[1], xb[p][src][1][0]);
        cmac(mc, mG[2], xb[p][src][2][0]); cmac(mc, mG[3], xb[p][src][3][0]);
    };
    int p = 0;

    auto fwd_row = [&](int j) {
        T t = Wr[j][0] * b[j][0];
#pragma unroll
        for (int c = 1; c < 5; ++c) cmac(t, Wr[j][c], b[j][c]);
        mc = t;
#pragma unroll
        for (int k = 0; k < 4; ++k) {
            T g = Zero<T>::v();
            cmsc(g, Wr[j][0], av[j][k]);
            cmsc(g, Wr[j][k + 1], dv[j][k]);
            mG[k] = g;
        }
    };
    fwd_row(0);
    T u[4];
    if constexpr (CH) {
        auto from_below = [&](T v) -> T { return seg == 4 ? row_shift4<true>(v) : lane_shift4<true>(v); };
        T zc = mc;
#pragma unroll 1
        for (int st = 1; st < seg; ++st) {
            const T up = from_below(zc);
            T t0 = mc, t1 = mG[1] * quad_bcast<1>(up);
            cmac(t0, mG[0], quad_bcast<0>(up)); cmac(t1, mG[3], quad_bcast<3>(up)); cmac(t0, mG[2], quad_bcast<2>(up));
            zc = (ch > 0) ? t0 + t1 : mc;
        }
        const T up = from_below(zc);
        u[0] = quad_bcast<0>(up); u[1] = quad_bcast<1>(up); u[2] = quad_bcast<2>(up); u[3] = quad_bcast<3>(up);
        if (ch == 0) { u[0] = Zero<T>::v(); u[1] = Zero<T>::v(); u[2] = Zero<T>::v(); u[3] = Zero<T>::v(); }
    } else {
#pragma unroll
    for (int j = 1; j < M; ++j) {
        publish(p);
        sync();
        fwd_row(j);
        compose_with(p, quad);
        p ^= 1;
    }
#pragma unroll 1
// ... 1 lines not shown
        publish(p);
        sync();
        if (ch >= st) { if (2 * st < seg) compose_with(p, quad - st); else compose_c_only(p, quad - st); }
        p ^= 1;
    }
    publish(p);
    sync();
#pragma unroll
    for (int k = 0; k < 4; ++k) u[k] = (ch > 0) ? xb[p][quad - 1][k][0] : Zero<T>::v();
    p ^= 1;
    }
    T z0[M], zr[M];
#pragma unroll
    for (int j = 0; j < M; ++j) {
        T y[5];
        y[0] = b[j][0];
#pragma unroll
        for (int k = 0; k < 4; ++k) {
            cmsc(y[0], u[k], av[j][k]);
            T t = b[j][k + 1];
            cmsc(t, u[k], dv[j][k]);
            y[k + 1] = t;
        }
        z0[j] = W0[j][0] * y[0];
        zr[j] = Wr[j][0] * y[0];
#pragma unroll
        for (int c = 1; c < 5; ++c) { cmac(z0[j], W0[j][c], y[c]); cmac(zr[j], Wr[j][c], y[c]); }
        if (j + 1 < M) { u[0] = quad_bcast<0>(zr[j]); u[1] = quad_bcast<1>(zr[j]); u[2] = quad_bcast<2>(zr[j]); u[3] = quad_bcast<3>(zr[j]); }
    }

    QPL_TS(4);
    auto bwd_row = [&](int j) {
        const double ar = (r == 0) ? av[j][0] : (r == 1) ? av[j][1] : (r == 2) ? av[j][2] : av[j][3];
        const double dr = (r == 0) ? dv[j][0] : (r == 1) ? dv[j][1] : (r == 2) ? dv[j][2] : dv[j][3];
        T g = z0[j] * ar;
        cmac(g, zr[j], dr);
        mc = g;
#pragma unroll
        for (int l = 0; l < 4; ++l) {
            T h = Zero<T>::v();
            cmsc(h, W0[j][l + 1], ar);
            cmsc(h, Wr[j][l + 1], dr);
            mG[l] = h;
        }
    };
    bwd_row(M - 1);
    T v[4];
    if constexpr (CH) {
        auto from_above = [&](T w) -> T { return seg == 4 ? row_shift4<false>(w) : lane_shift4<false>(w); };
        T vc = mc;
        const bool inner = ch + 1 < seg;
#pragma unroll 1
        for (int st = 1; st < seg; ++st) {
            const T dn = from_above(vc);
            T t0 = mc, t1 = mG[1] * quad_bcast<1>(dn);
            cmac(t0, mG[0], quad_bcast<0>(dn)); cmac(t1, mG[3], quad_bcast<3>(dn)); cmac(t0, mG[2], quad_bcast<2>(dn));
            vc = inner ? t0 + t1 : mc;
        }
        const T dn = from_above(vc);
        v[0] = quad_bcast<0>(dn); v[1] = quad_bcast<1>(dn); v[2] = quad_bcast<2>(dn); v[3] = quad_bcast<3>(dn);
        if (!inner) { v[0] = Zero<T>::v(); v[1] = Zero<T>::v(); v[2] = Zero<T>::v(); v[3] = Zero<T>::v(); }
    } else {
#pragma unroll
    for (int j = M - 2; j >= 0; --j) {
        publish(p);
        sync();
        bwd_row(j);
        compose_with(p, quad);
        p ^= 1;
    }
#pragma unroll 1
    for (int st = 1; st < seg; st <<= 1) {
        publish(p);
        sync();
        if (ch + st < seg) { if (2 * st < seg) compose_with(p, quad + st); else compose_c_only(p, quad + st); }
        p ^= 1;
    }
    publish(p);
    sync();
#pragma unroll
    for (int k = 0; k < 4; ++k) v[k] = (ch + 1 < seg) ? xb[p][quad + 1][k][0] : Zero<T>::v();
    }
    QPL_TS(5);
    T* eo = (a.e + boff_);
#pragma unroll
    for (int j = M - 1; j >= 0; --j) {
        T x0 = z0[j], xr = zr[j];
#pragma unroll
        for (int l = 0; l < 4; ++l) { cmsc(x0, W0[j][l + 1], v[l]); cmsc(xr, Wr[j][l + 1], v[l]); }
        const int i = ch * M + j;
        if (live && inl[j]) {
            if (r == 0) eo[dS0[j]] = x0;
            if (!lastb[j]) eo[dS[j]] = xr;
        }
        if (j > 0) {
            const double ar = (r == 0) ? av[j][0] : (r == 1) ? av[j][1] : (r == 2) ? av[j][2] : av[j][3];
            const double dr = (r == 0) ? dv[j][0] : (r == 1) ? dv[j][1] : (r == 2) ? dv[j][2] : dv[j][3];
            T vr = x0 * ar;
            cmac(vr, xr, dr);
            v[0] = quad_bcast<0>(vr); v[1] = quad_bcast<1>(vr); v[2] = quad_bcast<2>(vr); v[3] = quad_bcast<3>(vr);
        }
    }
    QPL_TS(6);
    };

    if constexpr (!HL) {
        one((u32)wg * (u32)lpg + (u32)(quad >> lseg), (u32)((a.mode == 0) ? a.cntA * a.cntB : a.cnt), (u32)a.t, (u32)a.jQ0);
#ifdef EMG3D_LAB
        if ((a.tile & 512) && blockIdx.x == 0 && threadIdx.x == 0) {
            asm volatile("s_waitcnt vmcnt(0)" ::: "memory");
            const long long tend = (long long)__builtin_readcyclecounter();
            printf("[qpl<%d,%d> seg %d lines %lld] args %lld loads issued %lld loads in + coefficients %lld forward %lld backward %lld stores issued %lld stores done %lld (cycles after entry)\n",
                   NW, M, seg, (long long)(a.cntA * a.cntB), qts[1] - qts[0], qts[2] - qts[0], qts[3] - qts[0], qts[4] - qts[0], qts[5] - qts[0], qts[6] - qts[0], tend - qts[0]);
        }
#endif
    } else {
        const int nPm = (int)a.rs.nP - 1, nQm = (int)a.rs.nQ - 1;
        const int tmin = (int)a.t, tmax = (int)a.jQ0;
        for (int th = tmin; th <= tmax; ++th) {
            const int tt = a.cnt ? tmax - (th - tmin) : th;
            const int lo = tt - nPm;
            int jq0 = lo <= 0 ? 1 : (lo + 1) / 2;
            if (jq0 < 1) jq0 = 1;
            int jq1 = (tt - 1) / 2;
            if (jq1 > nQm) jq1 = nQm;
            const int n = jq1 - jq0 + 1;
            for (int base = 0; base < n; base += lpg) {
                one((u32)(quad >> lseg), (u32)min(n - base, lpg), (u32)tt, (u32)(jq0 + base));
                __threadfence_block();
                __syncthreads();
            }
        }
    }
#undef QPL_TS
}
```

### emg3d_amd/csrc/stencil.hpp

```cpp
#pragma once
#include "common.hpp"

#define EMG_BLOCK 256

template <class T>
struct ResidualArgs {
    i64 nC[3];
    FieldLayout fl;
    T* r;
    const T* s;
    const T* e;
    const T* eta[3];
    const double* zeta;
    const double* h[3];
    const double* ih[3];
    double* partials;
    Batch bt;
    int xcd = 0;
    unsigned nbx = 0;
    int xs = 0;
};
HD i64 xmap(int xs, i64 v, i64 n) { return xs ? psplit(v, n) : v; }

template <class A>
__device__ __forceinline__ bool res_block_map(const A& a, unsigned& bx, unsigned& bz) {
    bx = blockIdx.x; bz = blockIdx.y;
    if (a.xcd == 1) {
        const unsigned nbx = gridDim.x, tot = nbx * gridDim.y, w = blockIdx.y * nbx + blockIdx.x;
        const unsigned c = w & 7u, per = tot >> 3, rem = tot & 7u;
        const unsigned slot = c * per + (c < rem ? c : rem) + (w >> 3);
        bz = slot / nbx;
        bx = slot - bz * nbx;
    } else if (a.xcd == 2) {
        const unsigned c = blockIdx.x & 7u, b0 = (c * a.nbx) >> 3, b1 = ((c + 1) * a.nbx) >> 3;
        bx = b0 + (blockIdx.x >> 3);
        if (bx >= b1) return false;
    }
    return true;
}

template <class T, int MODE>
__global__ __launch_bounds__(EMG_BLOCK) void k_residual(ResidualArgs<T> a) {
    EMG_ARGS_BURST(EMG_S(a.nC[0]), EMG_S(a.nC[1]), EMG_S(a.nC[2]), EMG_S(a.r), EMG_S(a.s), EMG_S(a.e), EMG_S(a.eta[0]), EMG_S(a.eta[1]),
                   EMG_S(a.eta[2]), EMG_S(a.zeta), EMG_S(a.h[0]), EMG_S(a.h[1]), EMG_S(a.h[2]), EMG_S(a.ih[0]), EMG_S(a.ih[1]), EMG_S(a.ih[2]),
                   EMG_S(a.partials), EMG_S(a.bt.st), EMG_S(a.bt.mask), EMG_S(a.xcd), EMG_S(a.nbx), EMG_S(a.xs), EMG_S(a.fl.off[1]),
                   EMG_S(a.fl.off[2]));
    EMG_BATCH(z, a.bt);
    T* const r_ = a.r + boff_;
    const T* const s_ = a.s + boff_;
    const i64 nx = a.nC[0], ny = a.nC[1], nz = a.nC[2];
    const i64 nNx = nx + 1, nNy = ny + 1;
    unsigned bx, bz;
    if (!res_block_map(a, bx, bz)) return;
    const i64 lin = (i64)bx * EMG_BLOCK + threadIdx.x;
    const i64 iz = bz;
    i64 ix, iy;
    unlin2(lin, nNx, ix, iy);
    double acc = 0.0;
    if (iy < nNy) {
        const FieldLayout& f = a.fl;
        const T* e = a.e + boff_;
#define EX(i, j, k) e[f.off[0] + xmap(a.xs, (i), nx) * f.st[0][0] + (j) * f.st[0][1] + (k) * f.st[0][2]]
#define EY(i, j, k) e[f.off[1] + xmap(a.xs, (i), nNx) * f.st[1][0] + (j) * f.st[1][1] + (k) * f.st[1][2]]
#define EZ(i, j, k) e[f.off[2] + xmap(a.xs, (i), nNx) * f.st[2][0] + (j) * f.st[2][1] + (k) * f.st[2][2]]
#define ZT(i, j, k) a.zeta[(i) + nx * ((j) + ny * (k))]
#define CI(i, j, k) ((i) + nx * ((j) + ny * (k)))
        const bool incell = (ix < nx) && (iy < ny) && (iz < nz);
        T ax = Zero<T>::v(), ay = Zero<T>::v(), az = Zero<T>::v();
        if (incell) {
            const i64 ixm = ix > 0 ? ix - 1 : 0, ixp = ix + 1;
            const i64 iym = iy > 0 ? iy - 1 : 0, iyp = iy + 1;
            const i64 izm = iz > 0 ? iz - 1 : 0, izp = iz + 1;
            const double hx = a.ih[0][ix], hxm = a.ih[0][ixm];
            const double hy = a.ih[1][iy], hym = a.ih[1][iym];
            const double hz = a.ih[2][iz], hzm = a.ih[2][izm];
            const T ex000 = EX(ix, iy, iz), ey000 = EY(ix, iy, iz), ez000 = EZ(ix, iy, iz);

            T v1pp = (EZ(ix, iyp, iz) - ez000) * hy - (EY(ix, iy, izp) - ey000) * hz;
            T v1mp = (ez000 - EZ(ix, iym, iz)) * hym - (EY(ix, iym, izp) - EY(ix, iym, iz)) * hz;
            T v1pm = (EZ(ix, iyp, izm) - EZ(ix, iy, izm)) * hy - (ey000 - EY(ix, iy, izm)) * hzm;
            T v2pp = (EX(ix, iy, izp) - ex000) * hz - (EZ(ixp, iy, iz) - ez000) * hx;
            T v2mp = (EX(ixm, iy, izp) - EX(ixm, iy, iz)) * hz - (ez000 - EZ(ixm, iy, iz)) * hxm;
            T v2pm = (ex000 - EX(ix, iy, izm)) * hzm - (EZ(ixp, iy, izm) - EZ(ix, iy, izm)) * hx;
            T v3pp = (EY(ixp, iy, iz) - ey000) * hx - (EX(ix, iyp, iz) - ex000) * hy;
// ... 684 lines not shown
        out[i] = eta_of((b * vol[i]) * sigma[i], T());
}
__device__ __forceinline__ double eta_eps_of(double p, double sig, double t, double) { return p * (sig - t); }
__device__ __forceinline__ c128 eta_eps_of(double p, double sig, double t, c128) { return mk(p * t, p * sig); }
template <class T>
__global__ __launch_bounds__(EMG_BLOCK) void k_eta_vs_eps(T* __restrict__ out, const double* __restrict__ vol,
                                                         const double* __restrict__ sigma, const double* __restrict__ epsr,
                                                         double b, double c, i64 n) {
    for (i64 i = (i64)blockIdx.x * EMG_BLOCK + threadIdx.x; i < n; i += (i64)gridDim.x * EMG_BLOCK) {
        const double p = b * vol[i];
        double t = c * epsr[i];
        asm volatile("" : "+v"(t));
        out[i] = eta_eps_of(p, sigma[i], t, T());
    }
}

template <class U, int SPLIT>
__global__ __launch_bounds__(256) void k_transpose01(U* __restrict__ dst, const U* __restrict__ src, i64 a0, i64 a1,
                                                     int nz, Batch bt) {
    __shared__ U tile[32][33];
    int z = blockIdx.z;
    if (bt.st) {
        const int b = z / nz;
        z -= b * nz;
        if (bt.mask && !bt.mask[b]) return;
        dst += (i64)b * bt.st; src += (i64)b * bt.st;
    }
    const i64 plane = a0 * a1 * (i64)z;
    const i64 i0 = (i64)blockIdx.x * 32, j0 = (i64)blockIdx.y * 32;
    for (int jj = threadIdx.y; jj < 32; jj += 8) {
        const i64 i = i0 + threadIdx.x, j = j0 + jj;
        if (i < a0 && j < a1) tile[jj][threadIdx.x] = src[plane + ((SPLIT < 0 || SPLIT == 2) ? psplit(i, a0) : i) + a0 * j];
    }
    __syncthreads();
    for (int ii = threadIdx.y; ii < 32; ii += 8) {
        const i64 j = j0 + threadIdx.x, i = i0 + ii;
        if (i < a0 && j < a1) dst[plane + (SPLIT > 0 ? psplit(j, a1) : j) + a1 * i] = tile[threadIdx.x][ii];
    }
}

struct FieldTransArgs {
    i64 off[3], a0[3], a1[3];
    int nz[3];
};
template <class U>
__global__ __launch_bounds__(256) void k_transpose01_field(U* __restrict__ dst, const U* __restrict__ src, FieldTransArgs t,
                                                           Batch bt) {
    __shared__ U tile[32][33];
    int z = blockIdx.z, c = 0;
    if (bt.st) {
        const int nzt = t.nz[0] + t.nz[1] + t.nz[2], b = z / nzt;
        z -= b * nzt;
        if (bt.mask && !bt.mask[b]) return;
        dst += (i64)b * bt.st; src += (i64)b * bt.st;
    }
    if (z >= t.nz[0]) { z -= t.nz[0]; c = 1; }
    if (c == 1 && z >= t.nz[1]) { z -= t.nz[1]; c = 2; }
    const i64 a0 = t.a0[c], a1 = t.a1[c];
    const i64 i0 = (i64)blockIdx.x * 32, j0 = (i64)blockIdx.y * 32;
    if (i0 >= a0 || j0 >= a1) return;
    const i64 plane = t.off[c] + a0 * a1 * (i64)z;
    for (int jj = threadIdx.y; jj < 32; jj += 8) {
        const i64 i = i0 + threadIdx.x, j = j0 + jj;
        if (i < a0 && j < a1) tile[jj][threadIdx.x] = src[plane + i + a0 * j];
    }
    __syncthreads();
    for (int ii = threadIdx.y; ii < 32; ii += 8) {
        const i64 j = j0 + threadIdx.x, i = i0 + ii;
        if (i < a0 && j < a1) dst[plane + j + a1 * i] = tile[threadIdx.x][ii];
    }
}

template <class U, int DIR>
__global__ __launch_bounds__(EMG_BLOCK) void k_split0(U* __restrict__ dst, const U* __restrict__ src, i64 n0, i64 rows,
                                                      Batch bt) {
    EMG_BATCH(y, bt); dst += boff_; src += boff_;
    const i64 n = n0 * rows;
    for (i64 t = (i64)blockIdx.x * EMG_BLOCK + threadIdx.x; t < n; t += (i64)gridDim.x * EMG_BLOCK) {
        const i64 row = t / n0, i = t - row * n0;
        if (DIR > 0) dst[row * n0 + psplit(i, n0)] = src[t];
        else dst[t] = src[row * n0 + psplit(i, n0)];
    }
}
```

### emg3d_amd/csrc/sweep_launch.hpp

```cpp
#pragma once
#include "smooth.hpp"
#include "stencil.hpp"

template <class T> void qc_launch(int stages, int lpw, bool zsep, bool big, dim3 grid, hipStream_t st, const LineArgs<T>& a);

template <class T> void thm_launch(int stages, int lpw, bool lifo, bool zsep, dim3 grid, hipStream_t st, const LineArgs<T>& a);
template <class T> void thm_lifo_attrs();

template <class T> void tha_launch(int helpers, bool zsep, dim3 grid, size_t dyn_lds, hipStream_t st, const LineArgs<T>& a);
template <class T> bool tha_attrs(int max_dyn_lds);

template <class T> void qpl_launch(int nw, int m, bool hl, int dm, bool chain, dim3 grid, hipStream_t st, const LineArgs<T>& a);

template <class T> void residual_launch(int mode, int kz, dim3 grid, hipStream_t st, const ResidualArgs<T>& a);
```

### emg3d_amd/csrc/sweep_plan.hpp

```cpp
#pragma once
#include <algorithm>
#include <cstdint>
#include <cstdio>
#include <cstdlib>

typedef int64_t i64;

#ifndef LAB_ENV
#ifdef EMG3D_LAB
inline long long lab_env_(const char* name, long long def) { const char* v = getenv(name); return v ? atoll(v) : def; }
inline int lab_env_ch_(const char* name) { const char* v = getenv(name); return v ? v[0] : 0; }
#define LAB_ENV(name, def) lab_env_(name, (long long)(def))
#define LAB_ENV_CH(name) lab_env_ch_(name)
#else
#define LAB_ENV(name, def) ((long long)(def))
#define LAB_ENV_CH(name) 0
#endif
#endif

constexpr int SWEEP_THA_LPW = 8, SWEEP_THA_RING = 8, SWEEP_THA_MAX_DYN_LDS = 140 * 1024, SWEEP_THA_STATIC_LDS = 18 * 1024;
inline i64 sweep_tha_lds_bytes(i64 nL, int tsize) {
    return (2 * SWEEP_THA_RING * 5 + 2 * ((nL + 1) / 2 + 2)) * (5 * SWEEP_THA_LPW) * (i64)tsize;
}

struct SweepKnobs {
    i64 simds = 1024;
    i64 lds_limit = 160 * 1024;
    bool tha_lds_granted = true;
    int order = 1, nsys = 1;
    int batch_tune = getenv("EMG3D_BATCH_TUNE") ? atoi(getenv("EMG3D_BATCH_TUNE")) : 0;

    int sweep_kernel = LAB_ENV_CH("EMG3D_SWEEP") == 't' ? 1 : 0;
    bool use_xt = LAB_ENV("EMG3D_XT", 1) != 0;
    i64 xt_min_cells = LAB_ENV("EMG3D_XT_MIN", 8192);
    int th_lpw = (int)LAB_ENV("EMG3D_TH_LPW", 0);
    int force_lpw = (int)LAB_ENV("EMG3D_LPW", 0);
    bool use_twist = LAB_ENV("EMG3D_TWIST", 1) != 0;
    i64 twist_max_lines_env = LAB_ENV("EMG3D_TWIST_MAX", 0);
    int tw_stages = (int)LAB_ENV("EMG3D_TW_STAGES", 0);
    int use_split = (int)LAB_ENV("EMG3D_SPLIT", 2);
    i64 split_min_cells = LAB_ENV("EMG3D_SPLIT_MIN_CELLS", 2000000);
    int use_q = (int)LAB_ENV("EMG3D_Q", 1);
    i64 q_min_lines_env = LAB_ENV("EMG3D_Q_MIN_LINES", 0);
    int q_stages = (int)LAB_ENV("EMG3D_Q_STAGES", 0);
    int q_lpw = (int)LAB_ENV("EMG3D_Q_LPW", 0);
    int q_big_lab = (int)LAB_ENV("EMG3D_Q_BIG", 0);
    int use_qpl = (int)LAB_ENV("EMG3D_QPL", 7);
    i64 qpl_min_nl = LAB_ENV("EMG3D_QPL_MIN", 2);
    i64 qpl_max_nl = LAB_ENV("EMG3D_QPL_MAX_NL", 64);
    i64 qpl_m2_min = LAB_ENV("EMG3D_QPL_M2", 32);
    int qpl_chain_seg = (int)LAB_ENV("EMG3D_QPL_CHAIN", 4);
    i64 qpl_few_lines_env = LAB_ENV("EMG3D_QPL_FEW", 0);
    i64 qpl_max_lines = LAB_ENV("EMG3D_QPL_MAX", (i64)1 << 40);
    int use_qdesc = (int)LAB_ENV("EMG3D_QDESC", 1);
    i64 qdesc_max_threads_env = LAB_ENV("EMG3D_QDESC_MAX", 0);
    int use_tha = (int)LAB_ENV("EMG3D_THA", 3);
    i64 tha_min_nl = LAB_ENV("EMG3D_THA_MIN", 33), tha_mid_nl = LAB_ENV("EMG3D_THA_MID", 64), tha_min_lines_env = LAB_ENV("EMG3D_THA_MIN_LINES", 0);
    i64 tha_max_nl = LAB_ENV("EMG3D_THA_MAX", 128);
    i64 tha_big_max_lines_env = LAB_ENV("EMG3D_THA_BIG_LINES", 0);
    int tha_split = (int)LAB_ENV("EMG3D_THA_SPLIT", 0);

    i64 q_min_lines() const { return q_min_lines_env > 0 ? q_min_lines_env : 8 * simds; }
    i64 twist_max_lines() const { return twist_max_lines_env > 0 ? twist_max_lines_env : q_min_lines(); }
    i64 qpl_few_lines() const { return qpl_few_lines_env > 0 ? qpl_few_lines_env : simds; }
    i64 qdesc_max_threads() const { return qdesc_max_threads_env > 0 ? qdesc_max_threads_env : (9000 * simds + 1023) / 1024; }
    i64 tha_min_lines() const { return tha_min_lines_env > 0 ? tha_min_lines_env : (1100 * simds + 1023) / 1024; }
    i64 tha_big_max_lines() const { return tha_big_max_lines_env > 0 ? tha_big_max_lines_env : (i64)SWEEP_THA_LPW * (simds / 4); }
};

struct SweepShape {
    i64 nC[3];
    int tsize;
    i64 cells() const { return nC[0] * nC[1] * nC[2]; }
    i64 edges() const {
        return nC[0] * (nC[1] + 1) * (nC[2] + 1) + (nC[0] + 1) * nC[1] * (nC[2] + 1) + (nC[0] + 1) * (nC[1] + 1) * nC[2];
    }
    i64 lines(int dir) const { return (nC[dir == 0 ? 1 : 0] / 2) * (nC[dir == 2 ? 1 : 2] / 2); }
    i64 lines_tot(int dir) const { return (nC[dir == 0 ? 1 : 0] - 1) * (nC[dir == 2 ? 1 : 2] - 1); }
    i64 field_stride(int c, int ax, bool transposed) const {
        const i64 d0 = (c == 0) ? nC[0] : nC[0] + 1, d1 = (c == 1) ? nC[1] : nC[1] + 1;
        return ax == 2 ? d0 * d1 : ((ax == 0) != transposed) ? 1 : (transposed ? d1 : d0);
    }
    i64 cell_stride(int ax, bool transposed) const {
        return ax == 2 ? nC[0] * nC[1] : ((ax == 0) != transposed) ? 1 : (transposed ? nC[1] : nC[0]);
    }
};

enum class SweepFamily { tpl, rp, qc, qc_big, thm, tha, qpl, qpl_chain };

inline void sweep_kernel_name(char* out, size_t len, SweepFamily f, int tsize, int p1 = 0, int p2 = 0) {
    static const char* const base[] = {"k_line_sweep", "k_line_sweep_rp", "k_line_sweep_qc", "k_line_sweep_qc_big", "k_line_sweep_thm",
                                       "k_line_sweep_tha", "k_line_sweep_qpl", "k_line_sweep_qpl_chain"};
    const char* tn = tsize == 16 ? "c128" : "f64";
    if (f == SweepFamily::tpl) snprintf(out, len, "%s<%s>", base[(int)f], tn);
    else if (f == SweepFamily::rp || f == SweepFamily::tha) snprintf(out, len, "%s<%s,%d>", base[(int)f], tn, p1);
    else snprintf(out, len, "%s<%s,%d,%d>", base[(int)f], tn, p1, p2);
}

struct SweepPlan {
    SweepFamily family = SweepFamily::tpl;
    int stages = 0, inst_lpw = 0, helpers = 0, NW = 0, M = 0, seg = 0;
    int qlpw = 0;
    bool big = false;
    bool split = false;
    bool xt = false;
    int work_id = 0;
    int fac_kind = 0;
    i64 fac_entries = 0;
    i64 mid = 0;
    bool qdesc = false;
    i64 nmax = 0;
    i64 lpw = 0;
    i64 rounds = 0;
    char name[64] = "";
};

inline bool sweep_wide_fits(const SweepKnobs& K, const SweepShape& G) {
    const i64 lim = (i64)1 << 32;
    const i64 mx = std::max(G.lines_tot(0), std::max(G.lines_tot(1), G.lines_tot(2)));
    return K.sweep_kernel == 0 && mx * 15 * (i64)G.tsize < lim && G.cells() * 8 < lim;
}
inline bool sweep_q_big_lines(const SweepKnobs& K, const SweepShape& G) {
    for (int d = 0; d < 3; ++d) if (G.lines(d) < std::max<i64>(K.q_min_lines(), 1)) return false;
    return K.order == 1 && K.use_q >= 1;
}
inline bool sweep_q_big(const SweepKnobs& K, const SweepShape& G) {
    return sweep_wide_fits(K, G) && sweep_q_big_lines(K, G) && (K.q_big_lab || G.edges() * (i64)G.tsize >= ((i64)1 << 32));
}
inline bool sweep_rp_fits(const SweepKnobs& K, const SweepShape& G) {
    return sweep_wide_fits(K, G) && G.edges() * (i64)G.tsize < ((i64)1 << 32) && !(K.q_big_lab && sweep_q_big_lines(K, G));
}
inline bool sweep_split_on(const SweepKnobs& K, const SweepShape& G) {
    return (K.use_split == 1 || (K.use_split == 2 && K.order == 1 && G.cells() >= K.split_min_cells)) &&
           (sweep_rp_fits(K, G) || sweep_q_big(K, G));
}

inline int sweep_tha_helpers(const SweepKnobs& K, const SweepShape& G, int dir) {
    if ((K.use_tha != 3 && K.use_tha != 2) || K.order != 1 || K.sweep_kernel != 0 || !K.use_twist || !sweep_rp_fits(K, G)) return 0;
// ... 12 lines not shown
    const i64 nL = G.nC[dir], cap = (nL >= K.qpl_m2_min) ? 256 : 128;
    i64 lines = G.lines(dir), max_nl = K.qpl_max_nl;
    if (K.batch_tune && K.nsys > 1 && K.order == 1) {
        lines *= K.nsys;
        max_nl = std::max<i64>(4, K.qpl_max_nl / K.nsys);
    }
    const i64 maxnl = (K.order == 0 || lines <= K.qpl_few_lines()) ? cap : std::min<i64>(max_nl, cap);
    if (nL < K.qpl_min_nl || nL > maxnl || !sweep_rp_fits(K, G)) return false;
    return lines <= K.qpl_max_lines;
}
inline bool sweep_twist_ok(const SweepKnobs& K, const SweepShape& G, int dir, bool q_on, bool transposed) {
    if (q_on || !K.use_twist || !sweep_rp_fits(K, G) || G.nC[dir] < 3) return false;
    if (G.lines(dir) >= K.twist_max_lines()) return false;
    const i64 lim24 = (i64)1 << 24;
    i64 mxs = 15 * G.lines_tot(dir) * (i64)G.tsize;
    for (int c = 0; c < 3; ++c) mxs = std::max(mxs, G.field_stride(c, dir, transposed) * (i64)G.tsize);
    mxs = std::max(mxs, G.cell_stride(dir, transposed) * 8);
    const i64 fac_bytes = 15 * G.lines_tot(dir) * G.nC[dir] * (i64)G.tsize;
    return mxs < lim24 && G.nC[dir] < lim24 && fac_bytes < ((i64)1 << 32);
}
inline int sweep_balanced_lpw(const SweepKnobs& K, i64 lines) {
    const i64 rounds = std::max<i64>(1, (lines + 16 * K.simds - 1) / (16 * K.simds));
    const i64 lpw = (lines + K.simds * rounds - 1) / (K.simds * rounds);
    return (int)std::min<i64>(16, std::max<i64>(lpw, 8));
}

inline SweepPlan plan_sweep(const SweepKnobs& K, const SweepShape& G, int dir) {
    SweepPlan p;
    const i64 nL = G.nC[dir], nmax = G.lines(dir), S = K.simds;
    const bool rp_fits = sweep_rp_fits(K, G), qpl = sweep_qpl_on(K, G, dir);
    p.nmax = nmax;
    p.split = sweep_split_on(K, G);
    p.xt = dir == 0 && K.use_xt && G.cells() >= K.xt_min_cells && !qpl;
    p.work_id = p.split ? (dir == 0 ? 0 : 1) : (p.xt ? 2 : 3 + dir);
    p.big = sweep_q_big(K, G) && !rp_fits;
    p.helpers = sweep_tha_helpers(K, G, dir);
    const bool q_on = K.use_q >= 2 || (K.use_q == 1 && nmax >= K.q_min_lines());
    p.fac_kind = (!qpl && sweep_twist_ok(K, G, dir, q_on, p.xt)) ? 3 : (!qpl && (rp_fits || p.big) && q_on) ? 4 : 0;
    p.mid = p.fac_kind == 3 ? (nL - 1) / 2 : nL - 1;
    p.fac_entries = (p.fac_kind == 4 ? 11 : 15) * nL;
    int p1 = 0, p2 = 0;
    if (p.fac_kind == 3 && p.helpers) {
        p.family = SweepFamily::tha;
        p1 = p.helpers;
        p.lpw = SWEEP_THA_LPW; p.rounds = (((nmax + p.lpw - 1) / p.lpw) * K.nsys + S / 4 - 1) / (S / 4);
    } else if (p.fac_kind == 3) {
        p.family = SweepFamily::thm;
        const i64 lines = nmax * K.nsys, r8 = (2 * ((lines + 7) / 8) + S - 1) / S, r12 = (2 * ((lines + 11) / 12) + S - 1) / S;
        p.inst_lpw = (K.th_lpw == 4 || K.th_lpw == 8 || K.th_lpw == 12) ? K.th_lpw : (23 * r12 < 20 * r8) ? 12 : 8;
        p.stages = K.tw_stages ? K.tw_stages : 3;
        p1 = p.stages; p2 = p.inst_lpw;
        p.lpw = p.inst_lpw; p.rounds = (2 * ((nmax + p.lpw - 1) / p.lpw) * K.nsys + S - 1) / S;
    } else if (qpl) {
        p.M = (nL >= K.qpl_m2_min) ? 2 : 1;
        p.seg = 4; while (p.seg < (nL + p.M - 1) / p.M) p.seg *= 2;
        p.NW = p.seg <= 16 ? 1 : p.seg / 16;
        p.family = (p.NW == 1 && p.M == 1 && K.order == 1 && p.seg <= K.qpl_chain_seg) ? SweepFamily::qpl_chain : SweepFamily::qpl;
        p1 = p.NW; p2 = p.M;
        p.fac_entries = 15 * (i64)p.M * p.seg;
        p.lpw = (16 * p.NW) / p.seg; p.rounds = (((nmax + p.lpw - 1) / p.lpw) * p.NW * K.nsys + S - 1) / S;
        p.qdesc = K.use_qdesc && K.order == 1 && p.NW == 1 && G.lines_tot(dir) * p.fac_entries < ((i64)1 << 32) &&
                  ((nmax + p.lpw - 1) / p.lpw) * 64 <= K.qdesc_max_threads();
    } else if ((rp_fits || p.big) && p.fac_kind == 4) {
        p.family = p.big ? SweepFamily::qc_big : SweepFamily::qc;
        p.inst_lpw = p.big ? 16 : K.q_lpw ? K.q_lpw : (nmax >= K.q_min_lines() ? 16 : 4);
        p.stages = (K.q_stages == 2 || K.q_stages == 3) ? K.q_stages
                 : (p.inst_lpw == 16 && nmax * K.nsys > 15 * S && nmax * K.nsys <= 16 * S) ? 2 : 3;
        p.qlpw = p.inst_lpw == 16 ? sweep_balanced_lpw(K, nmax * K.nsys) : p.inst_lpw;
        p1 = p.stages; p2 = p.inst_lpw;
        p.lpw = p.qlpw; p.rounds = (((nmax + p.lpw - 1) / p.lpw) * K.nsys + S - 1) / S;
    } else if (rp_fits || p.big) {
        p.family = SweepFamily::rp;
        p.lpw = K.force_lpw ? K.force_lpw : (nmax >= 8 * S ? 8 : 4);
        p.inst_lpw = (p.lpw == 8 || p.lpw == 12) ? (int)p.lpw : 4;
        p1 = p.inst_lpw;
        p.rounds = (((nmax + p.lpw - 1) / p.lpw) * K.nsys + S - 1) / S;
    } else {
        p.family = SweepFamily::tpl;
        p.lpw = 64; p.rounds = (((nmax + 63) / 64) * K.nsys + S - 1) / S;
    }
    sweep_kernel_name(p.name, sizeof p.name, p.family, G.tsize, p1, p2);
    return p;
}
```

### emg3d_amd/csrc/sweep_qpl.hip

```cpp
#include "sweep_launch.hpp"
#ifndef EMG3D_UNIT_T
#define EMG3D_UNIT_T 2
#endif
#include "smooth_qpl.hpp"

template <class T, int NW, int M>
static void qpl_launch_c(dim3 grid, hipStream_t st, const LineArgs<T>& a) {
    hipLaunchKernelGGL((k_line_sweep_qpl<T, NW, M>), grid, dim3(64 * NW), 0, st, a);
}
template <class T, int NW>
static void qpl_launch_hl(dim3 grid, hipStream_t st, const LineArgs<T>& a) {
    hipLaunchKernelGGL((k_line_sweep_qpl<T, NW, 1, true>), grid, dim3(64 * NW), 0, st, a);
}
template <class T, int M>
static void qpl_launch_m(int nw, int dm, bool chain, dim3 grid, hipStream_t st, const LineArgs<T>& a) {
    if constexpr (M == 1) {
        if (chain && dm != 1 && nw == 1) {
            if (dm == 2) hipLaunchKernelGGL((k_line_sweep_qpl<T, 1, 1, false, 2, true>), grid, dim3(64), 0, st, a);
            else hipLaunchKernelGGL((k_line_sweep_qpl<T, 1, 1, false, 0, true>), grid, dim3(64), 0, st, a);
            return;
        }
    }
    if (dm == 1) hipLaunchKernelGGL((k_line_sweep_qpl<T, 1, M, false, 1>), grid, dim3(64), 0, st, a);
    else if (dm == 2) hipLaunchKernelGGL((k_line_sweep_qpl<T, 1, M, false, 2>), grid, dim3(64), 0, st, a);
    else if (nw == 1) qpl_launch_c<T, 1, M>(grid, st, a);
    else if (nw == 2) qpl_launch_c<T, 2, M>(grid, st, a);
    else if (nw == 4) qpl_launch_c<T, 4, M>(grid, st, a);
    else qpl_launch_c<T, 8, M>(grid, st, a);
}
template <class T>
void qpl_launch(int nw, int m, bool hl, int dm, bool chain, dim3 grid, hipStream_t st, const LineArgs<T>& a) {
    if (hl) {
        if (nw == 1) qpl_launch_hl<T, 1>(grid, st, a);
        else if (nw == 2) qpl_launch_hl<T, 2>(grid, st, a);
        else if (nw == 4) qpl_launch_hl<T, 4>(grid, st, a);
        else qpl_launch_hl<T, 8>(grid, st, a);
    } else if (m == 2) qpl_launch_m<T, 2>(nw, dm, false, grid, st, a);
    else qpl_launch_m<T, 1>(nw, dm, chain, grid, st, a);
}
#if EMG3D_UNIT_T != 1
template void qpl_launch<double>(int, int, bool, int, bool, dim3, hipStream_t, const LineArgs<double>&);
#endif
#if EMG3D_UNIT_T != 0
template void qpl_launch<c128>(int, int, bool, int, bool, dim3, hipStream_t, const LineArgs<c128>&);
#endif
```

### include/emg3d_hip.h

```cpp
#ifndef EMG3D_HIP_H
#define EMG3D_HIP_H

#include <stdint.h>

#ifdef __cplusplus
extern "C" {
#endif

#define EMG3D_HIP_ABI_VERSION 109
int emg3d_hip_version(void);
int emg3d_hip_device_count(int* count);
int emg3d_hip_set_device(int device);
int emg3d_hip_device_info(int device, char* name, int64_t* total_mem, int* cu_count);
int emg3d_hip_mem_info(int device, int64_t* free_bytes, int64_t* total_bytes);

int64_t emg3d_hip_release_cached(void);
int64_t emg3d_hip_cached_bytes(void);
int64_t emg3d_hip_cached_bytes_on(int device);


int emg3d_amat_x(int dtype, int64_t nx, int64_t ny, int64_t nz, void* r, const void* e,
                 const void* eta_x, const void* eta_y, const void* eta_z, const double* zeta,
                 const double* hx, const double* hy, const double* hz);

int emg3d_get_h_field(int dtype, int64_t nx, int64_t ny, int64_t nz, void* hfield, const void* efield,
                      const double* zeta, const double* hx, const double* hy, const double* hz,
                      double smu0_re, double smu0_im);

int emg3d_gauss_seidel(int dtype, int dir, int64_t nx, int64_t ny, int64_t nz, void* e,
                       const void* s, const void* eta_x, const void* eta_y, const void* eta_z,
                       const double* zeta, const double* hx, const double* hy, const double* hz,
                       int nu, int order);

int emg3d_restrict(int dtype, int64_t nx, int64_t ny, int64_t nz, int64_t cnx, int64_t cny,
                   int64_t cnz, void* cr, const void* r, const double* const* w, int sc_dir);

int emg3d_restrict_weights(const double* vectorN, const double* vectorCC, const double* h,
                           int64_t nh, const double* cvectorN, const double* cvectorCC,
                           const double* ch, int64_t n, double* wl, double* w0, double* wr);

int emg3d_solve(int dtype, void* amat, void* bvec, int64_t n);

int emg3d_blocks_to_amat(int dtype, void* amat, void* bvec, int64_t n, const void* middle,
                         const double* left, const void* rhs, int64_t im, int64_t nC);

int emg3d_prolongation(int dtype, int64_t nx, int64_t ny, int64_t nz, const double* hx,
                       const double* hy, const double* hz, const double* origin, void* e,
                       const void* ce, int sc_dir);

int emg3d_restrict_model(int is_complex, int64_t nx, int64_t ny, int64_t nz, void* cparam,
                         const void* param, int sc_dir);

int emg3d_sweep_plan(int dtype, int64_t nx, int64_t ny, int64_t nz, int dir, int order, int nsys, int cu_count, char* name,
                     int64_t* info);

typedef struct emg3d_mg emg3d_mg_t;

int emg3d_mg_create(emg3d_mg_t** out, int dtype, int64_t nx, int64_t ny, int64_t nz,
                    const double* hx, const double* hy, const double* hz, const double* origin,
                    const void* eta_x, const void* eta_y, const void* eta_z, const double* zeta,
                    int device);
int emg3d_mg_create_sv(emg3d_mg_t** out, int dtype, int64_t nx, int64_t ny, int64_t nz, const double* hx,
                       const double* hy, const double* hz, const double* origin, const double* sv_x,
                       const double* sv_y, const double* sv_z, const double* zeta, double smu0_re,
                       double smu0_im, int device);

int emg3d_mg_create_vs(emg3d_mg_t** out, int dtype, int64_t nx, int64_t ny, int64_t nz, const double* hx,
                       const double* hy, const double* hz, const double* origin, const double* sigma_x,
                       const double* sigma_y, const double* sigma_z, const double* vol, const double* zeta,
                       double smu0_re, double smu0_im, int resistivity, int device);
int emg3d_mg_create_vse(emg3d_mg_t** out, int dtype, int64_t nx, int64_t ny, int64_t nz, const double* hx,
                        const double* hy, const double* hz, const double* origin, const double* sigma_x,
                        const double* sigma_y, const double* sigma_z, const double* vol, const double* zeta,
                        const double* epsilon_r, double smu0_re, double smu0_im, double seps0, int resistivity, int device);
void emg3d_mg_destroy(emg3d_mg_t* mg);

int emg3d_mg_set_params(emg3d_mg_t* mg, int cycle, int nu_init, int nu_pre, int nu_coarse,
                        int nu_post, const int* clevel, int order);

int emg3d_mg_set_sfield(emg3d_mg_t* mg, const void* sfield_host);
int emg3d_mg_set_sfield_vector(emg3d_mg_t* mg, const double* vector, double smu0_re, double smu0_im);
int emg3d_mg_set_sfield_dipole(emg3d_mg_t* mg, const double* src6, const double* scale6, int decimals,
                               int accumulate, double* sums3);
int emg3d_source_field(int dtype, int64_t nx, int64_t ny, int64_t nz, const double* hx, const double* hy,
                       const double* hz, const double* origin, const double* src6, const double* scale6,
                       int decimals, void* sfield, double* sums3);
int emg3d_mg_set_efield(emg3d_mg_t* mg, const void* efield_host);
int emg3d_mg_get_efield(emg3d_mg_t* mg, void* efield_host);
int emg3d_mg_get_residual(emg3d_mg_t* mg, void* rfield_host);
int emg3d_mg_get_hfield(emg3d_mg_t* mg, int use_zeta, double smu0_re, double smu0_im, void* hfield_host);

int emg3d_interp3d(int dtype, int64_t nx, int64_t ny, int64_t nz, const double* px, const double* py,
                   const double* pz, const void* values, int64_t n, const double* xi, int method, int has_fill,
                   double fill_value, double cval, void* out);
int emg3d_get_receiver_response(int dtype, int64_t nx, int64_t ny, int64_t nz, const double* hx, const double* hy,
                                const double* hz, const double* origin, const void* field, int is_electric,
                                int64_t n, const double* xyz, const double* factors, void* resp);
int emg3d_mg_get_receiver_response(emg3d_mg_t* mg, int magnetic, int use_zeta, double smu0_re, double smu0_im,
                                   int64_t n, const double* xyz, const double* factors, void* resp);

int emg3d_edges2cellaverages(int dtype, int64_t nx, int64_t ny, int64_t nz, const void* field, const double* vol,
                             void* out_x, void* out_y, void* out_z);
int emg3d_mg_gradient(emg3d_mg_t* mg, int efield_vec, double smu0_re, double smu0_im, double* grad);
int emg3d_mg_gradient3(emg3d_mg_t* mg, int efield_vec, double smu0_re, double smu0_im, double* grad_x, double* grad_y,
                       double* grad_z);

int emg3d_mg_grad_acc_reset(emg3d_mg_t* mg);
int emg3d_mg_grad_acc_add(emg3d_mg_t* mg, int fwd_bvec, double smu0_re, double smu0_im, const int32_t* use);
int emg3d_mg_grad_acc_get(emg3d_mg_t* mg, double* out);
int emg3d_mg_grad_acc3_reset(emg3d_mg_t* mg);
int emg3d_mg_grad_acc3_add(emg3d_mg_t* mg, int fwd_bvec, double smu0_re, double smu0_im, const int32_t* use);
int emg3d_mg_grad_acc3_get(emg3d_mg_t* mg, double* out_x, double* out_y, double* out_z);

int emg3d_cells2edges(int dtype, int64_t nx, int64_t ny, int64_t nz, const void* vx, const void* vy, const void* vz,
                      const double* vol, void* out_x, void* out_y, void* out_z);
int emg3d_mg_jvec_source(emg3d_mg_t* mg, int efield_vec, double smu0_re, double smu0_im, const double* vx, const double* vy,
                         const double* vz);
int emg3d_mg_jvec_source_b(emg3d_mg_t* mg, int fwd_bvec, double smu0_re, double smu0_im, const double* vx, const double* vy,
                           const double* vz, const int32_t* use);
int emg3d_mg_get_receiver_response_linear(emg3d_mg_t* mg, int64_t n, const double* xyz, const double* factors, void* resp);
int emg3d_mg_set_receiver_adjoint(emg3d_mg_t* mg, int64_t n, const double* xyz, const double* factors, const void* w,
                                  int accumulate);
int emg3d_mg_get_receiver_response_linear_h(emg3d_mg_t* mg, double smu0_re, double smu0_im, int64_t n, const double* xyz,
                                            const double* factors, void* resp);
int emg3d_mg_set_receiver_adjoint_ex(emg3d_mg_t* mg, int method, int magnetic, double smu0_re, double smu0_im, int64_t n,
                                     const double* xyz, const double* factors, const void* w, int accumulate);
int emg3d_mg_set_receiver_adjoint_b(emg3d_mg_t* mg, int method, int magnetic, double smu0_re, double smu0_im, int64_t n,
                                    const double* xyz, const double* factors, const void* w, const int32_t* use, int accumulate);
int emg3d_receiver_adjoint(int dtype, int64_t nx, int64_t ny, int64_t nz, const double* hx, const double* hy, const double* hz,
                           const double* origin, int is_electric, int method, double smu0_re, double smu0_im, int64_t n,
                           const double* xyz, const double* factors, const void* w, void* field);

int emg3d_volume_average_weights(const double* x1, int64_t n1, const double* x2, int64_t n2, double* w, int64_t* idx_in,
                                 int64_t* idx_out, int64_t* ptr, int64_t* nseg);
int emg3d_volume_average(int dtype, int64_t nx, int64_t ny, int64_t nz, const double* edges_x, const double* edges_y,
                         const double* edges_z, const void* values, int64_t mx, int64_t my, int64_t mz,
                         const double* new_edges_x, const double* new_edges_y, const double* new_edges_z, void* new_values,
// ... 68 lines not shown
```

Before: 249.6.

## Fuse colour-ordered line-sweep passes into one slab-tiled kernel with halo recompute

Colour-ordered line Gauss-Seidel passes are fused into a single kernel launch, used when the sweep plan is a qpl_chain with short segments. Each workgroup owns a slab along one axis, copies its slab plus halo into private scratch, and runs all passes on its shrinking live range. A scatter kernel then writes the owned region back to the field. This replaces one launch per colour pass and the global round trips between passes, at the cost of redundant halo work, per-slab scratch memory and an extra copy-in and scatter.

```diff
diff --git a/emg3d_amd/_lib.py b/emg3d_amd/_lib.py
--- a/emg3d_amd/_lib.py
+++ b/emg3d_amd/_lib.py
@@ -13,7 +13,7 @@
 c_double = ctypes.c_double
 c_dp = ctypes.POINTER(ctypes.c_double)
 
-ABI_VERSION = 109
+ABI_VERSION = 110
 
 SIGNATURES = {
     "emg3d_hip_version": (c_int, []),
@@ -36,6 +36,8 @@
     "emg3d_prolongation": (c_int, [c_int, c_i64, c_i64, c_i64, c_vp, c_vp, c_vp, c_vp, c_vp, c_vp, c_int]),
     "emg3d_restrict_model": (c_int, [c_int, c_i64, c_i64, c_i64, c_vp, c_vp, c_int]),
     "emg3d_sweep_plan": (c_int, [c_int, c_i64, c_i64, c_i64, c_int, c_int, c_int, c_int, ctypes.c_char_p, ctypes.POINTER(c_i64)]),
+    "emg3d_sweep_fuse_plan": (c_int, [c_int, c_i64, c_i64, c_i64, c_int, c_int, c_int, c_int, c_int, c_int, c_int, c_i64, ctypes.POINTER(c_i64),
+                                      ctypes.POINTER(c_i64), c_i64]),
     "emg3d_mg_create": (c_int, [ctypes.POINTER(c_vp), c_int, c_i64, c_i64, c_i64, c_vp, c_vp, c_vp, c_vp,
                                 c_vp, c_vp, c_vp, c_vp, c_int]),
     "emg3d_mg_destroy": (None, [c_vp]),
@@ -227,3 +229,21 @@
                                   1 if ordering == 'colour' else 0, int(nsys), int(cu_count), name, info), "emg3d_sweep_plan")
     return {"kernel": name.value.decode(), "lines_per_colour": info[0], "lines_per_wave": info[1], "rounds": info[2],
             "factor_kind": info[3], "split": bool(info[4]), "big_offsets": bool(info[5])}
+
+
+def sweep_fuse_plan(vnC, direction, npass, dtype=np.complex128, ordering='colour', nsys=1, cu_count=0, own=0, max_seg=0, budget=0):
+    info = (c_i64 * 8)()
+    cap = (4 + 2 * max(int(npass), 0)) * (max(vnC) + 1)
+    ranges = (c_i64 * cap)()
+    check(load().emg3d_sweep_fuse_plan(dtype_code(dtype), int(vnC[0]), int(vnC[1]), int(vnC[2]), int(direction),
+                                       1 if ordering == 'colour' else 0, int(nsys), int(cu_count), int(npass), int(own), int(max_seg), int(budget),
+                                       info, ranges, cap), "emg3d_sweep_fuse_plan")
+    out = {"fused": bool(info[0]), "axis": info[1], "nX": info[2], "own": info[3], "nslabs": info[4], "npass": info[5],
+           "waves": info[6], "scratch_bytes": info[7], "slabs": []}
+    if out["fused"]:
+        per = 4 + 2 * int(npass)
+        for k in range(info[4]):
+            r = ranges[per * k:per * (k + 1)]
+            out["slabs"].append({"own": (r[0], r[1]), "edges": (r[2], r[3]),
+                                 "live": [(r[4 + 2 * p], r[5 + 2 * p]) for p in range(int(npass))]})
+    return out
diff --git a/emg3d_amd/csrc/emg3d_hip.hip b/emg3d_amd/csrc/emg3d_hip.hip
--- a/emg3d_amd/csrc/emg3d_hip.hip
+++ b/emg3d_amd/csrc/emg3d_hip.hip
@@ -514,6 +514,36 @@
 }
 
 template <class T>
+static int fuse_plan_impl(i64 nx, i64 ny, i64 nz, int dir, int order, int nsys, int cu_count, int npass, int own, int max_seg, i64 budget, int64_t* info,
+                          int64_t* ranges, i64 nranges) {
+    SweepKnobs K;
+    if (cu_count > 0) K.simds = 4 * (i64)cu_count;
+    else sweep_device_knobs<T>(K, current_device());
+    K.order = order; K.nsys = nsys;
+    if (own > 0) K.fuse_own = own;
+    if (max_seg > 0) K.fuse_max_seg = max_seg;
+    if (budget > 0) K.fuse_max_bytes = budget;
+    const SweepShape G{{nx, ny, nz}, (int)sizeof(T)};
+    const FusePlan f = plan_fuse(K, G, dir - 1, npass);
+    int P, Q;
+    sweep_axes(dir - 1, P, Q);
+    info[0] = f.fused ? 1 : 0; info[1] = f.axis ? Q : P; info[2] = f.g.nX; info[3] = f.g.own; info[4] = f.g.nslabs; info[5] = f.g.npass;
+    info[6] = f.nw; info[7] = f.scratch_bytes;
+    if (!f.fused || !ranges) return 0;
+    const i64 per = 4 + 2 * (i64)npass;
+    if (nranges < per * f.g.nslabs) return -2;
+    for (int k = 0; k < f.g.nslabs; ++k) {
+        int64_t* r = ranges + per * k;
+        r[0] = fuse_x0(f.g, k); r[1] = fuse_x1(f.g, k);
+        i64 a = -1, b = -1;
+        for (int j = 0; j <= f.g.nX; ++j) if (fuse_owner(f.g, j) == k) { if (a < 0) a = j; b = j + 1; }
+        r[2] = a; r[3] = b;
+        for (int p = 0; p < npass; ++p) { r[4 + 2 * p] = fuse_lo(f.g, k, p); r[5 + 2 * p] = fuse_hi(f.g, k, p); }
+    }
+    return 0;
+}
+
+template <class T>
 static int jvec_stage(MG<T>* m, const double* const hv[3], const double* dv[3]) {
     Level<T>& L = *m->lv0;
     double* stage = reinterpret_cast<double*>(L.r);
@@ -844,6 +874,13 @@
                  : sweep_plan_impl<double>(nx, ny, nz, dir, order, nsys, cu_count, name, info);
 }
 
+int emg3d_sweep_fuse_plan(int dtype, int64_t nx, int64_t ny, int64_t nz, int dir, int order, int nsys, int cu_count, int npass, int own,
+                          int max_seg, int64_t budget, int64_t* info, int64_t* ranges, int64_t nranges) {
+    if (nx < 2 || ny < 2 || nz < 2 || dir < 1 || dir > 3 || order < 0 || order > 1 || nsys < 1 || nsys > 64 || npass < 0 || !info) return -2;
+    return dtype ? fuse_plan_impl<c128>(nx, ny, nz, dir, order, nsys, cu_count, npass, own, max_seg, budget, info, ranges, nranges)
+                 : fuse_plan_impl<double>(nx, ny, nz, dir, order, nsys, cu_count, npass, own, max_seg, budget, info, ranges, nranges);
+}
+
 int emg3d_mg_create(emg3d_mg_t** out, int dtype, int64_t nx, int64_t ny, int64_t nz, const double* hx,
                     const double* hy, const double* hz, const double* origin, const void* eta_x,
                     const void* eta_y, const void* eta_z, const double* zeta, int device) {
diff --git a/emg3d_amd/csrc/mg.hpp b/emg3d_amd/csrc/mg.hpp
--- a/emg3d_amd/csrc/mg.hpp
+++ b/emg3d_amd/csrc/mg.hpp
@@ -49,6 +49,11 @@
     T* fac[3] = {nullptr, nullptr, nullptr};
     void* qd[3][4] = {{nullptr, nullptr, nullptr, nullptr}, {nullptr, nullptr, nullptr, nullptr}, {nullptr, nullptr, nullptr, nullptr}};
     unsigned qdn[3][4] = {{0, 0, 0, 0}, {0, 0, 0, 0}, {0, 0, 0, 0}};
+    T* fz[3] = {nullptr, nullptr, nullptr};
+    i64 fz_n[3] = {0, 0, 0};
+    FusePlan fuse[3];
+    int fuse_key[3] = {-1, -1, -1};
+    std::vector<int> passes[3];
     i64 fac_lines[3] = {0, 0, 0};
     i64 fac_mid[3] = {0, 0, 0};
     int fac_kind[3] = {0, 0, 0};
@@ -1023,6 +1028,8 @@
             }
         }
         a.qd = nullptr; a.qdn = 0;
+        a.fe = nullptr; a.fnE = 0; a.fax = a.fnX = a.fown = a.fns = a.fnp = 0; a.fseq = 0;
+        for (int c = 0; c < 4; ++c) { a.fqd[c] = nullptr; a.fqdn[c] = 0; }
         a.qpl = P.NW; a.qM = P.M; a.seg = P.seg; a.qlpw = 0;
         a.tha = P.helpers;
         a.mode = 0; a.cP = a.cQ = 0; a.cntA = a.cntB = 0; a.t = a.jQ0 = a.cnt = 0;
@@ -1297,10 +1304,77 @@
         check_launch();
     }
 
+    void colour_passes(Level<T>& L, int dir, int nu, std::vector<int>& seq) {
+        int Pa, Qa;
+        sweep_axes(dir, Pa, Qa);
+        const i64 nP = L.nC[Pa], nQ = L.nC[Qa];
+        int iback = 0, last_c = -1;
+        seq.clear();
+        for (int it = 0; it < nu; ++it) {
+            iback = 1 - iback;
+            for (int ch = 0; ch < 4; ++ch) {
+                const int c = iback ? colour_perm_b[ch] : colour_perm[ch];
+                if (skip_idempotent && c == last_c) continue;
+                last_c = c;
+                if (((nP - (c & 1)) / 2) * ((nQ - (c >> 1)) / 2) <= 0) continue;
+                seq.push_back(c);
+            }
+        }
+    }
+    const FusePlan& ensure_fuse(Level<T>& L, int dir, int nu) {
+        const int key = nu * 256 + order + 2 * nsys;
+        if (L.fuse_key[dir] == key) return L.fuse[dir];
+        FusePlan& F = L.fuse[dir];
+        F = FusePlan();
+        L.fuse_key[dir] = key;
+        L.passes[dir].clear();
+        if (order != 1) return F;
+        colour_passes(L, dir, nu, L.passes[dir]);
+        const std::vector<int>& seq = L.passes[dir];
+        plan(L, dir);
+        F = plan_fuse(knobs, SweepShape{{L.nC[0], L.nC[1], L.nC[2]}, (int)sizeof(T)}, dir, (int)seq.size());
+        if (!F.fused) return F;
+        for (int c : seq) if (!L.qd[dir][c]) { F.fused = false; return F; }
+        const i64 need = (i64)nsys * F.g.nslabs * L.nE;
+        if (L.fz_n[dir] < need) {
+            T* z = try_alloc<T>(need);
+            if (!z) { F.fused = false; return F; }
+            if (L.fz[dir]) release(L.fz[dir]);
+            L.fz[dir] = z; L.fz_n[dir] = need;
+        }
+        return F;
+    }
+    void smooth_fused(Level<T>& L, int dir, const SweepPlan& P, const FusePlan& F, const std::vector<int>& seq, const LineArgs<T>& a) {
+        LineArgs<T> b = a;
+        b.mode = 0; b.xcd = 0;
+        b.fe = L.fz[dir]; b.fnE = L.nE; b.fax = F.axis;
+        b.fnX = F.g.nX; b.fown = F.g.own; b.fns = F.g.nslabs; b.fnp = F.g.npass;
+        b.fseq = 0;
+        for (int p = 0; p < F.g.npass; ++p) b.fseq |= (unsigned long long)seq[(size_t)p] << (4 * p);
+        for (int c = 0; c < 4; ++c) { b.fqd[c] = L.qd[dir][c]; b.fqdn[c] = L.qd[dir][c] ? L.qdn[dir][c] : 0u; }
+        if (log_launches) fprintf(stderr, "[sweep] nC %lld %lld %lld L %d lines %lld kernel %s split %d fused passes %d slabs %d own %d\n", (long long)a.nC[0],
+                                  (long long)a.nC[1], (long long)a.nC[2], a.L, (long long)a.nLinesTot, P.name, a.split, F.g.npass, F.g.nslabs, F.g.own);
+        memcpy(sweep_name, P.name, sizeof sweep_name);
+        if (broken) return;
+        qpl_fused_launch<T>(P.family == SweepFamily::qpl_chain, bgrid((unsigned)F.g.nslabs), stream, b);
+        ScatterArgs sa;
+        sa.nE = L.nE; sa.g = F.g;
+        int Pa, Qa;
+        sweep_axes(dir, Pa, Qa);
+        sa.ax = F.axis ? Qa : Pa;
+        for (int c = 0; c < 3; ++c) {
+            sa.off[c] = L.fl.off[c];
+            sa.d0[c] = (unsigned)((c == 0) ? L.nC[0] : L.nC[0] + 1); sa.d1[c] = (unsigned)((c == 1) ? L.nC[1] : L.nC[1] + 1);
+        }
+        hipLaunchKernelGGL(k_scatter_slabs<T>, dim3((unsigned)((L.nE + EMG_BLOCK - 1) / EMG_BLOCK), (unsigned)nsys), dim3(EMG_BLOCK), 0, stream,
+                           a.e, (const T*)L.fz[dir], sa, a.bt);
+    }
+
     void smooth_line(Level<T>& L, int dir, int nu, bool conv_in = true, bool conv_out = true) {
         if (nu <= 0) return;
         ensure_factor(L, dir);
         ensure_qdesc(L, dir);
+        const FusePlan& F = ensure_fuse(L, dir, nu);
         if (dry) { prepare_work(L, dir); return; }
         if (conv_in) to_work(L, dir);
         ensure_sflags(L, dir);
@@ -1309,24 +1383,21 @@
         const SweepPlan& P = plan(L, dir);
         const i64 nP = L.nC[a.P], nQ = L.nC[a.Q];
         const i64 nB[2] = {(nQ - 0) / 2, (nQ - 1) / 2};
+        if (order == 1) {
+            if (F.fused) smooth_fused(L, dir, P, F, L.passes[dir], a);
+            else for (int c : L.passes[dir]) {
+                a.mode = 0; a.cP = c & 1; a.cQ = c >> 1;
+                a.cntA = a.nA[a.cP]; a.cntB = nB[a.cQ];
+                a.rs.slot0 = (unsigned)a.base[c];
+                a.qd = L.qd[dir][c]; a.qdn = (L.qd[dir][c] ? L.qdn[dir][c] : 0u);
+                launch_sweep(P, a, a.cntA * a.cntB);
+            }
+            nu = 0;
+        }
         int iback = 0;
-        int last_c = -1;
         for (int it = 0; it < nu; ++it) {
             iback = 1 - iback;
-            if (order == 1) {
-                for (int ch = 0; ch < 4; ++ch) {
-                    const int c = iback ? colour_perm_b[ch] : colour_perm[ch];
-                    if (skip_idempotent && c == last_c) continue;
-                    last_c = c;
-                    a.mode = 0; a.cP = c & 1; a.cQ = c >> 1;
-                    a.cntA = a.nA[a.cP]; a.cntB = nB[a.cQ];
-                    a.rs.slot0 = (unsigned)a.base[c];
-                    a.qd = L.qd[dir][c]; a.qdn = (L.qd[dir][c] ? L.qdn[dir][c] : 0u);
-                    const i64 n = a.cntA * a.cntB;
-                    if (n <= 0) continue;
-                    launch_sweep(P, a, n);
-                }
-            } else {
+            {
                 const i64 tmin = 3, tmax = (nP - 1) + 2 * (nQ - 1);
                 if (lex_loop && a.qpl && a.qM == 1 && a.seg <= 16) {
                     LineArgs<T> b = a;
@@ -1613,7 +1684,7 @@
     void forget_factors() {
         auto clear = [](Level<T>& L) {
             for (int d = 0; d < 3; ++d) {
-                L.fac[d] = nullptr; L.fac_kind[d] = 0; L.plan_key[d] = -1;
+                L.fac[d] = nullptr; L.fac_kind[d] = 0; L.plan_key[d] = -1; L.fuse_key[d] = -1;
                 for (int c = 0; c < 4; ++c) { L.qd[d][c] = nullptr; L.qdn[d][c] = 0; }
             }
         };
diff --git a/emg3d_amd/csrc/smooth.hpp b/emg3d_amd/csrc/smooth.hpp
--- a/emg3d_amd/csrc/smooth.hpp
+++ b/emg3d_amd/csrc/smooth.hpp
@@ -39,6 +39,12 @@
     T* fac;
     const void* qd;
     unsigned qdn;
+    T* fe;
+    i64 fnE;
+    int fax, fnX, fown, fns, fnp;
+    unsigned long long fseq;
+    const void* fqd[4];
+    unsigned fqdn[4];
     i64 nLinesTot;
     i64 base[4];
     i64 nA[2];
diff --git a/emg3d_amd/csrc/smooth_qpl.hpp b/emg3d_amd/csrc/smooth_qpl.hpp
--- a/emg3d_amd/csrc/smooth_qpl.hpp
+++ b/emg3d_amd/csrc/smooth_qpl.hpp
@@ -1,5 +1,6 @@
 #pragma once
 #include "smooth.hpp"
+#include "sweep_plan.hpp"
 
 
 template <int K>
@@ -47,10 +48,11 @@
                  "s"(a.rs.nP), "s"(a.rs.nQ), "s"(a.qd), "s"(a.qdn));
 }
 
-template <class T, int NW, int M, bool HL = false, int DM = 0, bool CH = false>
+template <class T, int NW, int M, bool HL = false, int DM = 0, bool CH = false, bool FZ = false>
 __global__ __launch_bounds__(64 * NW) void k_line_sweep_qpl(LineArgs<T> a) {
-    static_assert(DM == 0 || (!HL && NW == 1), "descriptors: one wave per workgroup, colour order");
-    static_assert(!CH || (NW == 1 && M == 1 && !HL), "chain form: lines inside one wave, one block per quad");
+    static_assert(DM == 0 || (!HL && (NW == 1 || FZ)), "descriptors: one wave per workgroup, colour order");
+    static_assert(!CH || ((NW == 1 || FZ) && M == 1 && !HL), "chain form: lines inside one wave, one block per quad");
+    static_assert(!FZ || (DM == 2 && M == 1 && !HL), "fused passes: descriptors, one block per quad, colour order");
     constexpr int NQ = 16 * NW;
 #ifdef EMG3D_LAB
     long long qts[7] = {0, 0, 0, 0, 0, 0, 0};
@@ -69,32 +71,35 @@
     const int lpg = NQ >> lseg;
     typedef unsigned int u32;
     EMG_SWEEP_WG(a)
-    __shared__ T xb[2][NQ][4][5];
+    __shared__ T xb[2][(FZ && CH) ? 1 : NQ][4][5];
+    T* const ebase = FZ ? a.fe + ((i64)bsys_ * a.fns + wg) * a.fnE : a.e + boff_;
+    const void* qd_ = a.qd;
+    u32 qdn_ = a.qdn;
+    u32 tix = (u32)wg * (64u * NW) + (u32)tid;
     auto one = [&](const u32 gline, const u32 nlines, const u32 t_, const u32 jQ0_) {
     const bool live = gline < nlines;
     const int nL = (int)a.rs.nL;
     auto ld_d = [](const double* base, u32 idx) -> double { return *reinterpret_cast<const double*>(reinterpret_cast<const char*>(base) + idx * 8u); };
     auto ld_t = [](const T* base, u32 idx) -> T { return *reinterpret_cast<const T*>(reinterpret_cast<const char*>(base) + idx * (u32)sizeof(T)); };
-    const T* __restrict__ e = (a.e + boff_);
+    const T* __restrict__ e = ebase;
     const T* __restrict__ s = (a.s + boff_);
     T Wr[M][5], W0[M][5];
     T b[M][5];
     double av[M][4], dv[M][4];
     bool lastb[M], inl[M];
     u32 dS[M], dS0[M];
-    const u32 tix = (u32)wg * (64u * NW) + (u32)tid;
     constexpr int QD_U4 = 3, QD_D2 = 8;
     if constexpr (DM == 2) {
-        const uint4* const q4 = reinterpret_cast<const uint4*>(a.qd);
-        const emg_d2* const c2 = reinterpret_cast<const emg_d2*>(q4 + (size_t)(QD_U4 * M) * a.qdn);
+        const uint4* const q4 = reinterpret_cast<const uint4*>(qd_);
+        const emg_d2* const c2 = reinterpret_cast<const emg_d2*>(q4 + (size_t)(QD_U4 * M) * qdn_);
         uint4 u[M][QD_U4];
         emg_d2 cf[M][QD_D2];
 #pragma unroll
         for (int j = 0; j < M; ++j) {
 #pragma unroll
-            for (int k = 0; k < QD_U4; ++k) u[j][k] = q4[(u32)(QD_U4 * j + k) * a.qdn + tix];
-#pragma unroll
-            for (int k = 0; k < QD_D2; ++k) cf[j][k] = c2[(u32)(QD_D2 * j + k) * a.qdn + tix];
+            for (int k = 0; k < QD_U4; ++k) u[j][k] = q4[(u32)(QD_U4 * j + k) * qdn_ + tix];
+#pragma unroll
+            for (int k = 0; k < QD_D2; ++k) cf[j][k] = c2[(u32)(QD_D2 * j + k) * qdn_ + tix];
         }
         QPL_TS(2);
         T E[M][6], S[M], E0[M], S0[M];
@@ -290,7 +295,7 @@
     }
 
     QPL_TS(3);
-    auto sync = [&]() { if (NW > 1 && (HL || seg > 16)) __syncthreads(); else __builtin_amdgcn_wave_barrier(); };
+    auto sync = [&]() { if (!FZ && NW > 1 && (HL || seg > 16)) __syncthreads(); else __builtin_amdgcn_wave_barrier(); };
     T mc, mG[4];
     auto publish = [&](int p) {
         xb[p][quad][r][0] = mc;
@@ -458,7 +463,7 @@
     for (int k = 0; k < 4; ++k) v[k] = (ch + 1 < seg) ? xb[p][quad + 1][k][0] : Zero<T>::v();
     }
     QPL_TS(5);
-    T* eo = (a.e + boff_);
+    T* eo = ebase;
 #pragma unroll
     for (int j = M - 1; j >= 0; --j) {
         T x0 = z0[j], xr = zr[j];
@@ -480,7 +485,61 @@
     QPL_TS(6);
     };
 
-    if constexpr (!HL) {
+    if constexpr (FZ) {
+        const FuseGeom g{a.fnX, a.fown, a.fns, a.fnp};
+        const int k = (int)wg;
+        {
+            T* __restrict__ dst = ebase;
+            const T* __restrict__ src = a.e + boff_;
+            const int ra = fuse_lo(g, k, 0) - 1, rb = fuse_hi(g, k, 0) + 1;
+            const int X = a.fax ? 2 : 1;
+            const u32 nO = a.fax ? a.rs.nP : a.rs.nQ;
+#pragma unroll
+            for (int c = 0; c < 3; ++c) {
+                const u32 dL = a.rs.nL + (c != 0 ? 1u : 0u), dX = (u32)g.nX + (c != X ? 1u : 0u), dO = nO + ((c == 0 || c == X) ? 1u : 0u);
+                const int rbc = rb < (int)dX - 1 ? rb : (int)dX - 1;
+                if (rbc < ra) continue;
+                const u32 w = (u32)(rbc - ra + 1);
+                const u32 stL = a.rs.st[c][0], stX = a.fax ? a.rs.st[c][2] : a.rs.st[c][1], stO = a.fax ? a.rs.st[c][1] : a.rs.st[c][2];
+                const bool xf = stX < stL;
+                const u32 n0 = xf ? w : dL, n1 = xf ? dL : w, tot = n0 * n1 * dO;
+                for (u32 idx = (u32)tid; idx < tot; idx += 64u * NW) {
+                    const u32 t = idx / n0, i0 = idx - t * n0, i2 = t / n1, i1 = t - i2 * n1;
+                    const u32 iX = (u32)ra + (xf ? i0 : i1), iL = xf ? i1 : i0;
+                    const u32 off = a.rs.off[c] + iL * stL + iX * stX + i2 * stO;
+                    dst[off] = src[off];
+                }
+            }
+        }
+        __threadfence_block();
+        __syncthreads();
+        const u32 lslot = (u32)(quad >> lseg), wslot0 = (u32)(((tid >> 6) * 16) >> lseg);
+        for (int p = 0; p < g.npass; ++p) {
+            const int c = (int)((a.fseq >> (4 * p)) & 3ull);
+            const int cP = c & 1, cQ = c >> 1;
+            const u32 cA = (u32)a.nA[cP], cB = (u32)a.nB2[cQ];
+            const int cX = a.fax ? cQ : cP;
+            const u32 qa = (u32)(fuse_lo(g, k, p) - cX) >> 1, qb = (u32)(fuse_hi(g, k, p) + 1 - cX) >> 1;
+            const u32 nx = qb > qa ? qb - qa : 0u;
+            const u32 nloc = nx * (a.fax ? cA : cB);
+            qd_ = a.fqd[c]; qdn_ = a.fqdn[c];
+            for (u32 base = 0; base < nloc; base += (u32)lpg) {
+                if (base + wslot0 < nloc) {
+                    const u32 m = base + lslot;
+                    const bool lv = m < nloc;
+                    const u32 mm = lv ? m : base + wslot0;
+                    u32 qq, bq;
+                    if (a.fax == 0) { bq = mm / nx; qq = qa + (mm - bq * nx); }
+                    else { const u32 t = mm / cA; qq = mm - t * cA; bq = qa + t; }
+                    const u32 gl = bq * cA + qq;
+                    tix = ((gl >> (4 - lseg)) << 6) + ((((gl & ((16u >> lseg) - 1u)) << lseg) + (u32)ch) << 2) + (u32)r;
+                    one(lv ? 0u : 1u, 1u, 0u, 0u);
+                }
+            }
+            __threadfence_block();
+            __syncthreads();
+        }
+    } else if constexpr (!HL) {
         one((u32)wg * (u32)lpg + (u32)(quad >> lseg), (u32)((a.mode == 0) ? a.cntA * a.cntB : a.cnt), (u32)a.t, (u32)a.jQ0);
 #ifdef EMG3D_LAB
         if ((a.tile & 512) && blockIdx.x == 0 && threadIdx.x == 0) {
diff --git a/emg3d_amd/csrc/stencil.hpp b/emg3d_amd/csrc/stencil.hpp
--- a/emg3d_amd/csrc/stencil.hpp
+++ b/emg3d_amd/csrc/stencil.hpp
@@ -1,5 +1,6 @@
 #pragma once
 #include "common.hpp"
+#include "sweep_plan.hpp"
 
 #define EMG_BLOCK 256
 
@@ -850,3 +851,20 @@
         else dst[t] = src[row * n0 + psplit(i, n0)];
     }
 }
+
+struct ScatterArgs {
+    i64 nE, off[3];
+    unsigned d0[3], d1[3];
+    int ax;
+    FuseGeom g;
+};
+template <class T>
+__global__ __launch_bounds__(EMG_BLOCK) void k_scatter_slabs(T* __restrict__ e, const T* __restrict__ fe, ScatterArgs a, Batch bt) {
+    EMG_BATCH(y, bt);
+    const i64 idx = (i64)blockIdx.x * EMG_BLOCK + threadIdx.x;
+    if (idx >= a.nE) return;
+    const int c = idx >= a.off[2] ? 2 : idx >= a.off[1] ? 1 : 0;
+    const unsigned l = (unsigned)(idx - a.off[c]), q = l / a.d0[c], i0 = l - q * a.d0[c], i2 = q / a.d1[c], i1 = q - i2 * a.d1[c];
+    const int k = fuse_owner(a.g, (int)(a.ax == 0 ? i0 : a.ax == 1 ? i1 : i2));
+    e[boff_ + idx] = fe[((i64)b_ * a.g.nslabs + k) * a.nE + idx];
+}
diff --git a/emg3d_amd/csrc/sweep_launch.hpp b/emg3d_amd/csrc/sweep_launch.hpp
--- a/emg3d_amd/csrc/sweep_launch.hpp
+++ b/emg3d_amd/csrc/sweep_launch.hpp
@@ -11,5 +11,6 @@
 template <class T> bool tha_attrs(int max_dyn_lds);
 
 template <class T> void qpl_launch(int nw, int m, bool hl, int dm, bool chain, dim3 grid, hipStream_t st, const LineArgs<T>& a);
+template <class T> void qpl_fused_launch(bool chain, dim3 grid, hipStream_t st, const LineArgs<T>& a);
 
 template <class T> void residual_launch(int mode, int kz, dim3 grid, hipStream_t st, const ResidualArgs<T>& a);
diff --git a/emg3d_amd/csrc/sweep_plan.hpp b/emg3d_amd/csrc/sweep_plan.hpp
--- a/emg3d_amd/csrc/sweep_plan.hpp
+++ b/emg3d_amd/csrc/sweep_plan.hpp
@@ -54,6 +54,9 @@
     i64 qpl_max_lines = LAB_ENV("EMG3D_QPL_MAX", (i64)1 << 40);
     int use_qdesc = (int)LAB_ENV("EMG3D_QDESC", 1);
     i64 qdesc_max_threads_env = LAB_ENV("EMG3D_QDESC_MAX", 0);
+    int fuse_max_seg = (int)LAB_ENV("EMG3D_QPL_FUSE", 4);
+    i64 fuse_own = LAB_ENV("EMG3D_QPL_FUSE_W", 0);
+    i64 fuse_max_bytes = LAB_ENV("EMG3D_QPL_FUSE_BYTES", (i64)64 << 20);
     int use_tha = (int)LAB_ENV("EMG3D_THA", 3);
     i64 tha_min_nl = LAB_ENV("EMG3D_THA_MIN", 33), tha_mid_nl = LAB_ENV("EMG3D_THA_MID", 64), tha_min_lines_env = LAB_ENV("EMG3D_THA_MIN_LINES", 0);
     i64 tha_max_nl = LAB_ENV("EMG3D_THA_MAX", 128);
@@ -232,3 +235,46 @@
     sweep_kernel_name(p.name, sizeof p.name, p.family, G.tsize, p1, p2);
     return p;
 }
+
+constexpr int SWEEP_FUSE_MAX_PASSES = 16;
+#if defined(__HIPCC__)
+#define SWEEP_HD __host__ __device__
+#else
+#define SWEEP_HD
+#endif
+struct FuseGeom { int nX, own, nslabs, npass; };
+SWEEP_HD inline int fuse_x0(const FuseGeom& g, int k) { return 1 + k * g.own; }
+SWEEP_HD inline int fuse_x1(const FuseGeom& g, int k) { const int x = 1 + (k + 1) * g.own; return (k == g.nslabs - 1 || x > g.nX) ? g.nX : x; }
+SWEEP_HD inline int fuse_lo(const FuseGeom& g, int k, int p) { const int v = fuse_x0(g, k) - (g.npass - 1 - p); return v < 1 ? 1 : v; }
+SWEEP_HD inline int fuse_hi(const FuseGeom& g, int k, int p) { const int v = fuse_x1(g, k) + (g.npass - 1 - p); return v > g.nX - 1 ? g.nX - 1 : v; }
+SWEEP_HD inline int fuse_owner(const FuseGeom& g, int j) { const int k = j <= 0 ? 0 : (j - 1) / g.own; return k > g.nslabs - 1 ? g.nslabs - 1 : k; }
+
+struct FusePlan {
+    bool fused = false;
+    int axis = 0;
+    int nw = 0;
+    FuseGeom g = {0, 0, 0, 0};
+    i64 scratch_bytes = 0;
+};
+inline void sweep_axes(int dir, int& P, int& Q) { P = dir == 0 ? 1 : 0; Q = dir == 2 ? 1 : 2; }
+inline FusePlan plan_fuse(const SweepKnobs& K, const SweepShape& G, int dir, int npass) {
+    FusePlan f;
+    const SweepPlan p = plan_sweep(K, G, dir);
+    if (K.order != 1 || (p.family != SweepFamily::qpl && p.family != SweepFamily::qpl_chain) || p.NW != 1 || p.M != 1 || !p.qdesc) return f;
+    if (p.seg > K.fuse_max_seg || p.seg > 8 || npass < 3 || npass > SWEEP_FUSE_MAX_PASSES) return f;
+#ifndef EMG3D_LAB
+    if (p.family != SweepFamily::qpl_chain) return f;
+#endif
+    int P, Q;
+    sweep_axes(dir, P, Q);
+    f.axis = G.nC[Q] > G.nC[P] ? 1 : 0;
+    const i64 nX = G.nC[f.axis ? Q : P];
+    if (nX < 2 || nX > (1 << 20)) return f;
+    i64 own = K.fuse_own > 0 ? K.fuse_own : 2;
+    own = std::min<i64>(own, nX - 1);
+    f.g.nX = (int)nX; f.g.own = (int)own; f.g.nslabs = (int)((nX - 1 + own - 1) / own); f.g.npass = npass;
+    f.nw = p.family == SweepFamily::qpl_chain ? 8 : 4;
+    f.scratch_bytes = (i64)K.nsys * f.g.nslabs * G.edges() * (i64)G.tsize;
+    f.fused = f.scratch_bytes <= K.fuse_max_bytes;
+    return f;
+}
diff --git a/emg3d_amd/csrc/sweep_qpl.hip b/emg3d_amd/csrc/sweep_qpl.hip
--- a/emg3d_amd/csrc/sweep_qpl.hip
+++ b/emg3d_amd/csrc/sweep_qpl.hip
@@ -38,9 +38,18 @@
     } else if (m == 2) qpl_launch_m<T, 2>(nw, dm, false, grid, st, a);
     else qpl_launch_m<T, 1>(nw, dm, chain, grid, st, a);
 }
+template <class T>
+void qpl_fused_launch(bool chain, dim3 grid, hipStream_t st, const LineArgs<T>& a) {
+#ifdef EMG3D_LAB
+    if (!chain) { hipLaunchKernelGGL((k_line_sweep_qpl<T, 4, 1, false, 2, false, true>), grid, dim3(256), 0, st, a); return; }
+#endif
+    hipLaunchKernelGGL((k_line_sweep_qpl<T, 8, 1, false, 2, true, true>), grid, dim3(512), 0, st, a);
+}
 #if EMG3D_UNIT_T != 1
 template void qpl_launch<double>(int, int, bool, int, bool, dim3, hipStream_t, const LineArgs<double>&);
+template void qpl_fused_launch<double>(bool, dim3, hipStream_t, const LineArgs<double>&);
 #endif
 #if EMG3D_UNIT_T != 0
 template void qpl_launch<c128>(int, int, bool, int, bool, dim3, hipStream_t, const LineArgs<c128>&);
+template void qpl_fused_launch<c128>(bool, dim3, hipStream_t, const LineArgs<c128>&);
 #endif
diff --git a/include/emg3d_hip.h b/include/emg3d_hip.h
--- a/include/emg3d_hip.h
+++ b/include/emg3d_hip.h
@@ -7,7 +7,7 @@
 extern "C" {
 #endif
 
-#define EMG3D_HIP_ABI_VERSION 109
+#define EMG3D_HIP_ABI_VERSION 110
 int emg3d_hip_version(void);
 int emg3d_hip_device_count(int* count);
 int emg3d_hip_set_device(int device);
@@ -53,6 +53,9 @@
 
 int emg3d_sweep_plan(int dtype, int64_t nx, int64_t ny, int64_t nz, int dir, int order, int nsys, int cu_count, char* name,
                      int64_t* info);
+
+int emg3d_sweep_fuse_plan(int dtype, int64_t nx, int64_t ny, int64_t nz, int dir, int order, int nsys, int cu_count, int npass, int own,
+                          int max_seg, int64_t budget, int64_t* info, int64_t* ranges, int64_t nranges);
 
 typedef struct emg3d_mg emg3d_mg_t;
 
```

After: 252.7 (median of 6 runs). 1.2% higher.
